# YiZhiXiaoGuLI/xerus

Hardware: AMD Instinct MI355X
Metric: GFLOP/s on TT contraction + TT-round sweep time, order-10 rank-256 (higher is better)
Workload: dtype f64; 1 GPU; TT order-10 n=20 rank-256: <x,y> + x.round(256) per step; order=10, mode_size=20, rank=256, parallelism=replicas x1

## Files before the change

### include/xerus_amd.h

```cpp
#ifndef XERUS_AMD_H
#define XERUS_AMD_H

#include <stddef.h>
#include <stdint.h>

#ifdef __cplusplus
extern "C" {
#endif

typedef struct xrs_handle_s* xrs_handle_t;

#define XRS_OK 0
#define XRS_EINVAL (-1)
#define XRS_ENOMEM (-2)
#define XRS_EHIP (-3)
#define XRS_ENUMERIC 1

int xrs_create(xrs_handle_t* handle, int device);
int xrs_destroy(xrs_handle_t handle);
int xrs_set_stream(xrs_handle_t handle, void* hip_stream);
void* xrs_get_stream(xrs_handle_t handle);
int xrs_synchronize(xrs_handle_t handle);
const char* xrs_last_error(void);
const char* xrs_version(void);

int xrs_malloc(xrs_handle_t handle, void** ptr, size_t bytes);
int xrs_free(xrs_handle_t handle, void* ptr);
size_t xrs_pool_bytes(xrs_handle_t handle);
int xrs_upload(xrs_handle_t handle, double* dst_dev, const double* src_host, size_t n);
int xrs_download(xrs_handle_t handle, double* dst_host, const double* src_dev, size_t n);
int xrs_memset_zero(xrs_handle_t handle, double* dst_dev, size_t n);
int xrs_copy(xrs_handle_t handle, double* dst_dev, const double* src_dev, size_t n);

int xrs_nrm2(xrs_handle_t handle, double* result, const double* x, size_t n);
int xrs_dot(xrs_handle_t handle, double* result, const double* x, const double* y, size_t n);
int xrs_asum(xrs_handle_t handle, double* result, const double* x, size_t n);
int xrs_scal(xrs_handle_t handle, double* x, double alpha, size_t n);
int xrs_axpy(xrs_handle_t handle, double* y, double alpha, const double* x, size_t n);
int xrs_scale_rows(xrs_handle_t handle, double* X, const double* s, size_t m, size_t n);

int xrs_gemm(xrs_handle_t handle, double* C, size_t M, size_t N, double alpha,
             const double* A, size_t lda, int transA, size_t K,
             const double* B, size_t ldb, int transB);

int xrs_gemm_batched(xrs_handle_t handle, size_t count, double* const* C, size_t M, size_t N, double alpha,
                     const double* const* A, size_t lda, int transA, size_t K,
                     const double* const* B, size_t ldb, int transB);

int xrs_gemm_sym(xrs_handle_t handle, double* C, size_t N, double alpha,
                 const double* A, size_t lda, int transA, size_t K,
                 const double* B, size_t ldb, int transB);

int xrs_gemm_forms(xrs_handle_t handle, size_t count, double* const* C, size_t M, size_t N, double alpha,
                   const double* const* A, size_t lda, int transA, size_t K,
                   const double* const* B, size_t ldb, int transB, int sym, int tri);

int xrs_gemm_f32(xrs_handle_t handle, float* C, size_t M, size_t N, float alpha,
                 const float* A, size_t lda, int transA, size_t K,
                 const float* B, size_t ldb, int transB);

int xrs_permute(xrs_handle_t handle, double* out, const double* in, size_t ndim,
                const size_t* dims, const size_t* shuffle);

int xrs_qc(xrs_handle_t handle, double* Q, double* C, size_t* rank, const double* A, size_t m, size_t n);
int xrs_cq(xrs_handle_t handle, double* C, double* Q, size_t* rank, const double* A, size_t m, size_t n);
int xrs_qr(xrs_handle_t handle, double* Q, double* R, const double* A, size_t m, size_t n);
int xrs_rq(xrs_handle_t handle, double* R, double* Q, const double* A, size_t m, size_t n);
int xrs_svd(xrs_handle_t handle, double* U, double* S, double* Vt, const double* A, size_t m, size_t n);
int xrs_svd_batched(xrs_handle_t handle, double* U, double* S, double* Vt, int* status,
                    const double* A, size_t batch, size_t m, size_t n);
int xrs_svd_batched_fits(size_t m, size_t n);
int xrs_solve(xrs_handle_t handle, double* X, const double* A, size_t m, size_t n, const double* B, size_t p);
int xrs_solve_least_squares(xrs_handle_t handle, double* X, const double* A, size_t m, size_t n, const double* B, size_t p);
int xrs_svd_rows_vt(xrs_handle_t handle, double* S, double* Vt, int* sweeps, const double* A, size_t p, size_t q, int kernel);
int xrs_sym_tridiag(xrs_handle_t handle, double* d, double* e, const double* A, size_t n);
int xrs_sym_eig_top(xrs_handle_t handle, double* lam, double* Ut, int* status, const double* A, size_t n, size_t kk);


int xrs_tt_move_core(xrs_handle_t handle, size_t d, const size_t* n, size_t* r, double** cores,
                     int canonicalized, size_t core_position, size_t position, int keep_rank);
int xrs_tt_round(xrs_handle_t handle, size_t d, const size_t* n, size_t* r, double** cores,
                 int canonicalized, size_t core_position, const size_t* max_ranks, double eps);
int xrs_tt_soft_threshold(xrs_handle_t handle, size_t d, const size_t* n, size_t* r, double** cores,
                          int canonicalized, size_t core_position, const double* taus);
int xrs_tt_entrywise_product(xrs_handle_t handle, size_t d, const size_t* ext, const size_t* ra, const double* const* A,
                             const size_t* rb, const double* const* B, double alpha, double** out);
int xrs_tt_entrywise_square(xrs_handle_t handle, size_t d, const size_t* ext, const size_t* r, const double* const* A,
                            double alpha, double** out, size_t* r_out);
int xrs_tt_rank_one_argmax(xrs_handle_t handle, size_t d, const size_t* ext, const double* const* cores, size_t* pos);
int xrs_tt_operator_apply(xrs_handle_t handle, size_t d, const size_t* n, const size_t* m, const size_t* p, const size_t* ra,
                          const double* const* A, const size_t* rb, const double* const* B, int transpose_a, double** out);
#define XRS_ROUND_CHAIN 1
#define XRS_ROUND_TRUNCATE 2
#define XRS_ROUND_REFERENCE 3
#define XRS_ROUND_GENERAL 4
int xrs_tt_last_round_path(xrs_handle_t handle);
int xrs_tt_dot(xrs_handle_t handle, double* result, size_t d, const size_t* n,
               const size_t* rx, const double* const* xcores,
               const size_t* ry, const double* const* ycores);

int xrs_tt_dot_async(xrs_handle_t handle, size_t d, const size_t* n,
                     const size_t* rx, const double* const* xcores,
                     const size_t* ry, const double* const* ycores);
int xrs_tt_dot_wait(xrs_handle_t handle, double* result);
int xrs_tt_dot_f32(xrs_handle_t handle, double* result, size_t d, const size_t* n,
                   const size_t* rx, const double* const* xcores,
                   const size_t* ry, const double* const* ycores);

int xrs_tt_tangent_project(xrs_handle_t handle, size_t d, const size_t* n, const size_t* ru, const double* const* U,
                           const size_t* rz, const double* const* Z, double** V, double** UU, size_t* fallback_edges);
int xrs_tt_tangent_to_tt(xrs_handle_t handle, size_t d, const size_t* n, const size_t* r, const double* const* U,
                         const double* const* V, int add_base, double** out);
int xrs_tt_tangent_dot(xrs_handle_t handle, double* result, size_t d, const size_t* n, const size_t* r,
                       const double* const* UU, const double* const* A, const double* const* B);

typedef int (*xrs_allreduce_fn)(void* ctx, double* buf, size_t count);
typedef int (*xrs_allgather_fn)(void* ctx, const double* send, double* recv, size_t count);

typedef struct xrs_comm_s* xrs_comm_t;
int xrs_comm_unique_id(void* id128_out);
int xrs_comm_create(xrs_handle_t handle, int nranks, int rank, const void* id128, xrs_comm_t* comm_out);
int xrs_comm_destroy(xrs_comm_t comm);
size_t xrs_comm_calls(xrs_comm_t comm);
int xrs_comm_allreduce(void* comm, double* buf, size_t count);
int xrs_comm_emulate(xrs_handle_t handle, int nranks, xrs_comm_t* comm_out);
int xrs_comm_allgather(void* comm, const double* send, double* recv, size_t count);

int xrs_tt_gather_sharded(xrs_handle_t handle, size_t d, const size_t* n_global, int world, int rank, const size_t* r,
                          const double* const* local_cores, double** full_cores_out, xrs_allgather_fn allgather, void* ctx);
int xrs_tt_shard(xrs_handle_t handle, size_t d, const size_t* n_global, int world, int rank, const size_t* r,
                 const double* const* full_cores, double** local_out);

int xrs_tt_round_sharded(xrs_handle_t handle, size_t d, const size_t* n_local, size_t* r, double** cores,
                         const size_t* max_ranks, double eps, xrs_allreduce_fn allreduce, void* ctx, int* certified);

int xrs_tt_round_sharded_ex(xrs_handle_t handle, size_t d, const size_t* n_local, size_t* r, double** cores,
                            const size_t* max_ranks, double eps, int world, int rank, xrs_allreduce_fn allreduce,
                            void* ctx, int* path);

int xrs_tt_dot_sharded(xrs_handle_t handle, double* result, size_t d, const size_t* n_local, const size_t* rx,
                       const double* const* X, const size_t* ry, const double* const* Y, xrs_allreduce_fn allreduce,
                       void* ctx);

int xrs_uq_basis(xrs_handle_t handle, double* P, const double* xi, size_t N, size_t n);
int xrs_uq_stack_congruence(xrs_handle_t handle, double* Lout, const double* Lprev, const double* X, const double* P,
                            size_t N, size_t a, size_t n, size_t b);
int xrs_uq_quadform(xrs_handle_t handle, double* result, const double* L, const double* V, size_t N, size_t a);


int xrs_philox_words(xrs_handle_t handle, uint32_t* out, size_t s, size_t q, uint64_t seed, uint32_t stream);
int xrs_gaussian_matrix(xrs_handle_t handle, double* G, size_t s, size_t m, uint64_t seed, uint32_t stream);
#define XRS_SKETCH_FUSED 1
#define XRS_SKETCH_MATERIALISED 2
int xrs_sketch_gaussian(xrs_handle_t handle, double* Y, size_t s, const double* A, size_t m, size_t n, uint64_t seed,
                        uint32_t stream, int route);
int xrs_sketch_last_route(xrs_handle_t handle);


int xrs_als_local_apply(xrs_handle_t handle, double* y, const double* x, size_t rl, size_t n, size_t rr, size_t pl,
                        size_t pr, const double* L, const double* A, const double* R, int normal);
#define XRS_CG_CONVERGED 0
#define XRS_CG_MAX_ITER 1
#define XRS_CG_BREAKDOWN 2
int xrs_als_local_cg(xrs_handle_t handle, double* x, const double* b, size_t rl, size_t n, size_t rr, size_t pl,
                     size_t pr, const double* L, const double* A, const double* R, int normal, double tol,
                     size_t max_iter, size_t check_every, size_t* iters, double* relres, int* status);

#define XRS_EIG_CONVERGED 0
#define XRS_EIG_MAX_ITER 1
#define XRS_EIG_BREAKDOWN 2
int xrs_als_local_eig(xrs_handle_t handle, double* x, size_t rl, size_t n, size_t rr, size_t pl, size_t pr,
                      const double* L, const double* A, const double* R, double tol, size_t max_iter, size_t check_every,
                      double* theta, size_t* iters, double* relres, int* status);
int xrs_geneig_lowest(int k, const double* G, const double* H, double* theta, double* c);

#define XRS_KFAM_GEMM 1u
#define XRS_KFAM_PERMUTE 2u
#define XRS_KFAM_QR 4u
#define XRS_KFAM_SVD 8u
#define XRS_KFAM_ELEMWISE 16u
#define XRS_KFAM_SPLITK 32u
int xrs_prof_begin(xrs_handle_t handle, uint32_t family_mask);
int xrs_prof_end(xrs_handle_t handle, size_t* launches, double* total_ms, double* flops, double* bytes);

#ifdef __cplusplus
}
#endif
#endif
```

### xerus_amd/capi.py

```python
from __future__ import annotations

import ctypes as C
import os
from typing import Sequence

import numpy as np

_HERE = os.path.dirname(os.path.abspath(__file__))
LIB_PATH = os.environ.get("XRS_LIB_PATH") or os.path.join(_HERE, "libxerus_amd.so")

_SZ = C.c_size_t
_DP = C.c_void_p

SIGNATURES = {
    "xrs_create": (C.c_int, [C.POINTER(_DP), C.c_int]),
    "xrs_destroy": (C.c_int, [_DP]),
    "xrs_set_stream": (C.c_int, [_DP, _DP]),
    "xrs_get_stream": (_DP, [_DP]),
    "xrs_synchronize": (C.c_int, [_DP]),
    "xrs_last_error": (C.c_char_p, []),
    "xrs_version": (C.c_char_p, []),
    "xrs_malloc": (C.c_int, [_DP, C.POINTER(_DP), _SZ]),
    "xrs_free": (C.c_int, [_DP, _DP]),
    "xrs_pool_bytes": (_SZ, [_DP]),
    "xrs_upload": (C.c_int, [_DP, _DP, _DP, _SZ]),
    "xrs_download": (C.c_int, [_DP, _DP, _DP, _SZ]),
    "xrs_memset_zero": (C.c_int, [_DP, _DP, _SZ]),
    "xrs_copy": (C.c_int, [_DP, _DP, _DP, _SZ]),
    "xrs_nrm2": (C.c_int, [_DP, C.POINTER(C.c_double), _DP, _SZ]),
    "xrs_dot": (C.c_int, [_DP, C.POINTER(C.c_double), _DP, _DP, _SZ]),
    "xrs_asum": (C.c_int, [_DP, C.POINTER(C.c_double), _DP, _SZ]),
    "xrs_scal": (C.c_int, [_DP, _DP, C.c_double, _SZ]),
    "xrs_axpy": (C.c_int, [_DP, _DP, C.c_double, _DP, _SZ]),
    "xrs_scale_rows": (C.c_int, [_DP, _DP, _DP, _SZ, _SZ]),
    "xrs_gemm": (C.c_int, [_DP, _DP, _SZ, _SZ, C.c_double, _DP, _SZ, C.c_int, _SZ, _DP, _SZ, C.c_int]),
    "xrs_gemm_f32": (C.c_int, [_DP, _DP, _SZ, _SZ, C.c_float, _DP, _SZ, C.c_int, _SZ, _DP, _SZ, C.c_int]),
    "xrs_gemm_sym": (C.c_int,[_DP, _DP, _SZ, C.c_double, _DP, _SZ, C.c_int, _SZ, _DP, _SZ, C.c_int]),
    "xrs_gemm_batched": (C.c_int, [_DP, _SZ, C.POINTER(_DP), _SZ, _SZ, C.c_double, C.POINTER(_DP), _SZ, C.c_int, _SZ,
                                   C.POINTER(_DP), _SZ, C.c_int]),
    "xrs_gemm_forms": (C.c_int, [_DP, _SZ, C.POINTER(_DP), _SZ, _SZ, C.c_double, C.POINTER(_DP), _SZ, C.c_int, _SZ,
                                 C.POINTER(_DP), _SZ, C.c_int, C.c_int, C.c_int]),
    "xrs_permute": (C.c_int, [_DP, _DP, _DP, _SZ, C.POINTER(_SZ), C.POINTER(_SZ)]),
    "xrs_qc": (C.c_int, [_DP, _DP, _DP, C.POINTER(_SZ), _DP, _SZ, _SZ]),
    "xrs_cq": (C.c_int, [_DP, _DP, _DP, C.POINTER(_SZ), _DP, _SZ, _SZ]),
    "xrs_qr": (C.c_int, [_DP, _DP, _DP, _DP, _SZ, _SZ]),
    "xrs_rq": (C.c_int, [_DP, _DP, _DP, _DP, _SZ, _SZ]),
    "xrs_svd": (C.c_int, [_DP, _DP, _DP, _DP, _DP, _SZ, _SZ]),
    "xrs_svd_batched": (C.c_int, [_DP, _DP, _DP, _DP, C.POINTER(C.c_int), _DP, _SZ, _SZ, _SZ]),
    "xrs_svd_batched_fits": (C.c_int, [_SZ, _SZ]),
    "xrs_solve": (C.c_int, [_DP, _DP, _DP, _SZ, _SZ, _DP, _SZ]),
    "xrs_solve_least_squares": (C.c_int, [_DP, _DP, _DP, _SZ, _SZ, _DP, _SZ]),
    "xrs_svd_rows_vt": (C.c_int, [_DP, _DP, _DP, C.POINTER(C.c_int), _DP, _SZ, _SZ, C.c_int]),
    "xrs_sym_eig_top": (C.c_int, [_DP, _DP, _DP, C.POINTER(C.c_int), _DP, _SZ, _SZ]),
    "xrs_sym_tridiag": (C.c_int, [_DP, _DP, _DP, _DP, _SZ]),
    "xrs_tt_entrywise_product": (C.c_int, [_DP, _SZ, C.POINTER(_SZ), C.POINTER(_SZ), C.POINTER(_DP), C.POINTER(_SZ), C.POINTER(_DP),
                                           C.c_double, C.POINTER(_DP)]),
    "xrs_tt_entrywise_square": (C.c_int, [_DP, _SZ, C.POINTER(_SZ), C.POINTER(_SZ), C.POINTER(_DP), C.c_double, C.POINTER(_DP),
                                          C.POINTER(_SZ)]),
    "xrs_tt_rank_one_argmax": (C.c_int, [_DP, _SZ, C.POINTER(_SZ), C.POINTER(_DP), C.POINTER(_SZ)]),
    "xrs_tt_operator_apply": (C.c_int, [_DP, _SZ, C.POINTER(_SZ), C.POINTER(_SZ), C.POINTER(_SZ), C.POINTER(_SZ), C.POINTER(_DP),
                                        C.POINTER(_SZ), C.POINTER(_DP), C.c_int, C.POINTER(_DP)]),
    "xrs_tt_move_core": (C.c_int, [_DP, _SZ, C.POINTER(_SZ), C.POINTER(_SZ), C.POINTER(_DP), C.c_int, _SZ, _SZ, C.c_int]),
    "xrs_tt_round": (C.c_int, [_DP, _SZ, C.POINTER(_SZ), C.POINTER(_SZ), C.POINTER(_DP), C.c_int, _SZ,
                               C.POINTER(_SZ), C.c_double]),
    "xrs_tt_dot": (C.c_int, [_DP, C.POINTER(C.c_double), _SZ, C.POINTER(_SZ), C.POINTER(_SZ), C.POINTER(_DP),
                             C.POINTER(_SZ), C.POINTER(_DP)]),
    "xrs_tt_dot_async": (C.c_int, [_DP, _SZ, C.POINTER(_SZ), C.POINTER(_SZ), C.POINTER(_DP), C.POINTER(_SZ),
                                   C.POINTER(_DP)]),
    "xrs_tt_dot_wait": (C.c_int, [_DP, C.POINTER(C.c_double)]),
    "xrs_tt_dot_f32": (C.c_int, [_DP, C.POINTER(C.c_double), _SZ, C.POINTER(_SZ), C.POINTER(_SZ), C.POINTER(_DP),
                                 C.POINTER(_SZ), C.POINTER(_DP)]),
    "xrs_tt_round_sharded": (C.c_int, [_DP, _SZ, C.POINTER(_SZ), C.POINTER(_SZ), C.POINTER(_DP), C.POINTER(_SZ),
                                       C.c_double, _DP, _DP, C.POINTER(C.c_int)]),
    "xrs_tt_round_sharded_ex": (C.c_int, [_DP, _SZ, C.POINTER(_SZ), C.POINTER(_SZ), C.POINTER(_DP), C.POINTER(_SZ),
                                          C.c_double, C.c_int, C.c_int, _DP, _DP, C.POINTER(C.c_int)]),
    "xrs_tt_dot_sharded": (C.c_int, [_DP, C.POINTER(C.c_double), _SZ, C.POINTER(_SZ), C.POINTER(_SZ), C.POINTER(_DP),
                                     C.POINTER(_SZ), C.POINTER(_DP), _DP, _DP]),
    "xrs_tt_tangent_project": (C.c_int, [_DP, _SZ, C.POINTER(_SZ), C.POINTER(_SZ), C.POINTER(_DP), C.POINTER(_SZ),
                                         C.POINTER(_DP), C.POINTER(_DP), C.POINTER(_DP), C.POINTER(_SZ)]),
    "xrs_tt_tangent_to_tt": (C.c_int, [_DP, _SZ, C.POINTER(_SZ), C.POINTER(_SZ), C.POINTER(_DP), C.POINTER(_DP), C.c_int,
                                       C.POINTER(_DP)]),
    "xrs_tt_tangent_dot": (C.c_int, [_DP, C.POINTER(C.c_double), _SZ, C.POINTER(_SZ), C.POINTER(_SZ), C.POINTER(_DP),
                                     C.POINTER(_DP), C.POINTER(_DP)]),
    "xrs_tt_last_round_path": (C.c_int, [_DP]),
    "xrs_tt_soft_threshold": (C.c_int, [_DP, _SZ, C.POINTER(_SZ), C.POINTER(_SZ), C.POINTER(_DP), C.c_int, _SZ,
                                        C.POINTER(C.c_double)]),
    "xrs_comm_unique_id": (C.c_int, [_DP]),
    "xrs_comm_create": (C.c_int, [_DP, C.c_int, C.c_int, _DP, C.POINTER(_DP)]),
    "xrs_comm_emulate": (C.c_int, [_DP, C.c_int, C.POINTER(_DP)]),
    "xrs_comm_destroy": (C.c_int, [_DP]),
    "xrs_comm_calls": (_SZ, [_DP]),
    "xrs_comm_allreduce": (C.c_int, [_DP, _DP, _SZ]),
    "xrs_comm_allgather": (C.c_int, [_DP, _DP, _DP, _SZ]),
    "xrs_tt_gather_sharded": (C.c_int, [_DP, _SZ, C.POINTER(_SZ), C.c_int, C.c_int, C.POINTER(_SZ), C.POINTER(_DP),
                                        C.POINTER(_DP), _DP, _DP]),
    "xrs_tt_shard": (C.c_int, [_DP, _SZ, C.POINTER(_SZ), C.c_int, C.c_int, C.POINTER(_SZ), C.POINTER(_DP), C.POINTER(_DP)]),
    "xrs_uq_basis": (C.c_int, [_DP, _DP, _DP, _SZ, _SZ]),
    "xrs_uq_stack_congruence": (C.c_int, [_DP, _DP, _DP, _DP, _DP, _SZ, _SZ, _SZ, _SZ]),
    "xrs_uq_quadform": (C.c_int, [_DP, C.POINTER(C.c_double), _DP, _DP, _SZ, _SZ]),
    "xrs_philox_words": (C.c_int, [_DP, _DP, _SZ, _SZ, C.c_uint64, C.c_uint32]),
    "xrs_gaussian_matrix": (C.c_int, [_DP, _DP, _SZ, _SZ, C.c_uint64, C.c_uint32]),
    "xrs_sketch_gaussian": (C.c_int, [_DP, _DP, _SZ, _DP, _SZ, _SZ, C.c_uint64, C.c_uint32, C.c_int]),
    "xrs_sketch_last_route": (C.c_int, [_DP]),
    "xrs_als_local_apply": (C.c_int, [_DP, _DP, _DP, _SZ, _SZ, _SZ, _SZ, _SZ, _DP, _DP, _DP, C.c_int]),
    "xrs_als_local_cg": (C.c_int, [_DP, _DP, _DP, _SZ, _SZ, _SZ, _SZ, _SZ, _DP, _DP, _DP, C.c_int, C.c_double, _SZ, _SZ,
                                   C.POINTER(_SZ), C.POINTER(C.c_double), C.POINTER(C.c_int)]),
    "xrs_als_local_eig": (C.c_int, [_DP, _DP, _SZ, _SZ, _SZ, _SZ, _SZ, _DP, _DP, _DP, C.c_double, _SZ, _SZ,
                                    C.POINTER(C.c_double), C.POINTER(_SZ), C.POINTER(C.c_double), C.POINTER(C.c_int)]),
    "xrs_geneig_lowest": (C.c_int, [C.c_int, C.POINTER(C.c_double), C.POINTER(C.c_double), C.POINTER(C.c_double),
                                    C.POINTER(C.c_double)]),
    "xrs_prof_begin": (C.c_int, [_DP, C.c_uint32]),
    "xrs_prof_end": (C.c_int, [_DP, C.POINTER(_SZ), C.POINTER(C.c_double), C.POINTER(C.c_double),
                               C.POINTER(C.c_double)]),
}

KFAM_GEMM, KFAM_PERMUTE, KFAM_QR, KFAM_SVD, KFAM_ELEMWISE, KFAM_SPLITK = 1, 2, 4, 8, 16, 32
ROUND_PATHS = {0: None, 1: "chain", 2: "truncate", 3: "reference", 4: "general"}
SKETCH_AUTO, SKETCH_FUSED, SKETCH_MATERIALISED = 0, 1, 2
SKETCH_ROUTES = {0: None, 1: "fused", 2: "materialised"}

_lib = None


class XrsError(RuntimeError):

    def __init__(self, fn: str, code: int, msg: str):
        super().__init__(f"{fn} failed with status {code}: {msg}")
        self.code = code


def load(path: str | None = None) -> C.CDLL:
    global _lib
    if _lib is not None and path is None:
        return _lib
    p = path or LIB_PATH
    if not os.path.exists(p):
        raise ImportError(f"{p} is missing: build it with `python -c 'import __graft_entry__ as g; g.build()'`")
    lib = C.CDLL(p)
    for name, (res, args) in SIGNATURES.items():
        f = getattr(lib, name)
        f.restype = res
        f.argtypes = args
    if path is None:
        _lib = lib
    return lib


def _check(fn: str, status: int):
    if status != 0:
        raise XrsError(fn, status, load().xrs_last_error().decode())


def svd_batched_fits(m: int, n: int) -> bool:
    return bool(load().xrs_svd_batched_fits(int(m), int(n)))


def geneig_lowest(k: int, G: Sequence[float], H: Sequence[float]):
    m = k * (k + 1) // 2
    if k not in (2, 3) or len(G) != m or len(H) != m:
        raise XrsError("xrs_geneig_lowest", -1, f"k = {k} needs {m} entries of each upper triangle")
    g, h = (C.c_double * m)(*[float(v) for v in G]), (C.c_double * m)(*[float(v) for v in H])
    theta, c = C.c_double(), (C.c_double * 3)()
    used = load().xrs_geneig_lowest(k, g, h, C.byref(theta), c)
    return used, theta.value, np.array(c[:k])


def _arr(vals: Sequence[int]):
    return (_SZ * len(vals))(*[int(v) for v in vals])


class Handle:

    def __init__(self, device: int = 0):
        self.lib = load()
        self.h = _DP()
        _check("xrs_create", self.lib.xrs_create(C.byref(self.h), device))

    def close(self):
        if self.h:
            _check("xrs_destroy", self.lib.xrs_destroy(self.h))
            self.h = _DP()

    def __del__(self):
        try:
            self.close()
        except Exception:
            pass

    def malloc(self, nbytes: int) -> int:
        p = _DP()
        _check("xrs_malloc", self.lib.xrs_malloc(self.h, C.byref(p), nbytes))
        return p.value or 0

    def free(self, ptr: int):
        _check("xrs_free", self.lib.xrs_free(self.h, _DP(ptr)))

    def pool_bytes(self) -> int:
        return int(self.lib.xrs_pool_bytes(self.h))

    def synchronize(self):
        _check("xrs_synchronize", self.lib.xrs_synchronize(self.h))

    def set_stream(self, stream_ptr: int | None):
        _check("xrs_set_stream", self.lib.xrs_set_stream(self.h, _DP(stream_ptr or 0)))

    def stream(self) -> int:
        return self.lib.xrs_get_stream(self.h) or 0

    def array(self, a: np.ndarray) -> "DeviceArray":
        return DeviceArray.from_host(self, a)

    def empty(self, shape) -> "DeviceArray":
        return DeviceArray(self, tuple(int(s) for s in shape))

    def zeros(self, shape) -> "DeviceArray":
        d = DeviceArray(self, tuple(int(s) for s in shape))
        _check("xrs_memset_zero", self.lib.xrs_memset_zero(self.h, _DP(d.ptr), d.size))
        return d

    def gemm(self, C_: "DeviceArray", M, N, alpha, A: "DeviceArray", lda, transA, K, B: "DeviceArray", ldb, transB):
        _check("xrs_gemm", self.lib.xrs_gemm(self.h, _DP(C_.ptr), M, N, alpha, _DP(A.ptr), lda, int(transA), K,
                                            _DP(B.ptr), ldb, int(transB)))

    def gemm_f32(self, C_: "Float32Array", M, N, alpha, A: "Float32Array", lda, transA, K, B: "Float32Array", ldb, transB):
        _check("xrs_gemm_f32", self.lib.xrs_gemm_f32(self.h, _DP(C_.ptr), M, N, float(alpha), _DP(A.ptr), lda, int(transA),
                                                    K, _DP(B.ptr), ldb, int(transB)))

    def array_f32(self, a: np.ndarray) -> "Float32Array":
        return Float32Array.from_host(self, a)

    def gemm_sym(self, C_: "DeviceArray", N, alpha, A: "DeviceArray", lda, transA, K, B: "DeviceArray", ldb, transB):
        _check("xrs_gemm_sym", self.lib.xrs_gemm_sym(self.h, _DP(C_.ptr), N, alpha, _DP(A.ptr), lda, int(transA), K,
                                                    _DP(B.ptr), ldb, int(transB)))

    def gemm_batched(self, Cs, M, N, alpha, As, lda, transA, K, Bs, ldb, transB):
        cnt = len(Cs)
        tab = lambda xs: (_DP * max(1, cnt))(*[_DP(x.ptr) for x in xs])
        _check("xrs_gemm_batched", self.lib.xrs_gemm_batched(self.h, cnt, tab(Cs), M, N, alpha, tab(As), lda, int(transA),
                                                            K, tab(Bs), ldb, int(transB)))

    def gemm_forms(self, Cs, M, N, alpha, As, lda, transA, K, Bs, ldb, transB, sym: bool = False, tri: int = 0):
        cnt = len(Cs)
        tab = lambda xs: (_DP * max(1, cnt))(*[_DP(x.ptr) for x in xs])
        _check("xrs_gemm_forms", self.lib.xrs_gemm_forms(self.h, cnt, tab(Cs), M, N, alpha, tab(As), lda, int(transA), K,
                                                        tab(Bs), ldb, int(transB), int(sym), int(tri)))

    def tangent_to_tt(self, n, r, Us, Vs, add_base: bool):
        d = len(n)
        tab = lambda xs: (_DP * d)(*[_DP(x.ptr) for x in xs])
        out = (_DP * d)()
        _check("xrs_tt_tangent_to_tt", self.lib.xrs_tt_tangent_to_tt(self.h, d, _arr(n), _arr(r), tab(Us), tab(Vs),
                                                                    int(add_base), out))
        cores = []
        for k in range(d):
            shape = (2 * r[k] if k else 1, n[k], 2 * r[k + 1] if k + 1 < d else 1)
            c = DeviceArray(self, shape, ptr=out[k])
            c.owned = True
            cores.append(c)
        return cores

    def matmul(self, A: "DeviceArray", transA: bool, B: "DeviceArray", transB: bool, alpha: float = 1.0):
        am, ak = (A.shape[1], A.shape[0]) if transA else (A.shape[0], A.shape[1])
        bk, bn = (B.shape[1], B.shape[0]) if transB else (B.shape[0], B.shape[1])
        assert ak == bk, (A.shape, B.shape)
        out = self.empty((am, bn))
        self.gemm(out, am, bn, alpha, A, A.shape[1], transA, ak, B, B.shape[1], transB)
        return out

    def permute(self, out: "DeviceArray", inp: "DeviceArray", dims, shuffle):
        _check("xrs_permute", self.lib.xrs_permute(self.h, _DP(out.ptr), _DP(inp.ptr), len(dims), _arr(dims),
                                                  _arr(shuffle)))

    def reshuffle(self, inp: "DeviceArray", shuffle):
        dims = inp.shape
        out_dims = [0] * len(dims)
        for i, s in enumerate(shuffle):
            out_dims[s] = dims[i]
        out = self.empty(tuple(out_dims))
        self.permute(out, inp, dims, shuffle)
        return out

    def nrm2(self, x: "DeviceArray") -> float:
        r = C.c_double()
        _check("xrs_nrm2", self.lib.xrs_nrm2(self.h, C.byref(r), _DP(x.ptr), x.size))
        return r.value

    def dot(self, x: "DeviceArray", y: "DeviceArray") -> float:
        r = C.c_double()
        _check("xrs_dot", self.lib.xrs_dot(self.h, C.byref(r), _DP(x.ptr), _DP(y.ptr), x.size))
        return r.value

    def asum(self, x: "DeviceArray") -> float:
        r = C.c_double()
        _check("xrs_asum", self.lib.xrs_asum(self.h, C.byref(r), _DP(x.ptr), x.size))
        return r.value

    def scal(self, x: "DeviceArray", alpha: float):
        _check("xrs_scal", self.lib.xrs_scal(self.h, _DP(x.ptr), alpha, x.size))

    def axpy(self, y: "DeviceArray", alpha: float, x: "DeviceArray"):
        _check("xrs_axpy", self.lib.xrs_axpy(self.h, _DP(y.ptr), alpha, _DP(x.ptr), x.size))

    def scale_rows(self, X: "DeviceArray", s: "DeviceArray"):
        _check("xrs_scale_rows", self.lib.xrs_scale_rows(self.h, _DP(X.ptr), _DP(s.ptr), X.shape[0], X.size // max(1, X.shape[0])))

    def qc(self, A: "DeviceArray"):
        m, n = A.shape
        k = min(m, n)
        Q, Cm = self.empty((m, k)), self.empty((k, n))
        r = _SZ()
        _check("xrs_qc", self.lib.xrs_qc(self.h, _DP(Q.ptr), _DP(Cm.ptr), C.byref(r), _DP(A.ptr), m, n))
        rank = r.value
        Q.shape, Cm.shape = (m, rank), (rank, n)
        return Q, Cm, rank

    def cq(self, A: "DeviceArray"):
        m, n = A.shape
        k = min(m, n)
        Cm, Q = self.empty((m, k)), self.empty((k, n))
        r = _SZ()
        _check("xrs_cq", self.lib.xrs_cq(self.h, _DP(Cm.ptr), _DP(Q.ptr), C.byref(r), _DP(A.ptr), m, n))
        rank = r.value
        Cm.shape, Q.shape = (m, rank), (rank, n)
        return Cm, Q, rank

    def qr(self, A: "DeviceArray"):
        m, n = A.shape
        k = min(m, n)
        Q, R = self.empty((m, k)), self.empty((k, n))
        _check("xrs_qr", self.lib.xrs_qr(self.h, _DP(Q.ptr), _DP(R.ptr), _DP(A.ptr), m, n))
        return Q, R

    def rq(self, A: "DeviceArray"):
        m, n = A.shape
        k = min(m, n)
        R, Q = self.empty((m, k)), self.empty((k, n))
        _check("xrs_rq", self.lib.xrs_rq(self.h, _DP(R.ptr), _DP(Q.ptr), _DP(A.ptr), m, n))
        return R, Q

    def svd(self, A: "DeviceArray"):
        m, n = A.shape
        k = min(m, n)
        U, S, Vt = self.empty((m, k)), self.empty((k,)), self.empty((k, n))
        _check("xrs_svd", self.lib.xrs_svd(self.h, _DP(U.ptr), _DP(S.ptr), _DP(Vt.ptr), _DP(A.ptr), m, n))
        return U, S, Vt

    def svd_batched(self, A: "DeviceArray", want_status: bool = True):
        batch, m, n = A.shape
        k = min(m, n)
        U, S, Vt = self.empty((batch, m, k)), self.empty((batch, k)), self.empty((batch, k, n))
        st = np.zeros(batch, dtype=np.intc) if want_status else None
        _check("xrs_svd_batched", self.lib.xrs_svd_batched(
            self.h, _DP(U.ptr), _DP(S.ptr), _DP(Vt.ptr), st.ctypes.data_as(C.POINTER(C.c_int)) if want_status else None,
            _DP(A.ptr), batch, m, n))
        return U, S, Vt, st

    def solve(self, A: "DeviceArray", B: "DeviceArray", least_squares: bool = False):
        m, n = A.shape
        p = B.shape[1] if len(B.shape) == 2 else 1
        X = self.empty((n, p) if len(B.shape) == 2 else (n,))
        fn = "xrs_solve_least_squares" if least_squares else "xrs_solve"
        _check(fn, getattr(self.lib, fn)(self.h, _DP(X.ptr), _DP(A.ptr), m, n, _DP(B.ptr), p))
        return X

    def sym_eig_top(self, A: "DeviceArray", kk: int):
        n = A.shape[0]
        lam, Ut, st = self.empty((kk,)), self.empty((kk, n)), C.c_int()
        _check("xrs_sym_eig_top", self.lib.xrs_sym_eig_top(self.h, _DP(lam.ptr), _DP(Ut.ptr), C.byref(st), _DP(A.ptr), n, kk))
        return lam, Ut, st.value

    def sym_tridiag(self, A: "DeviceArray"):
        n = A.shape[0]
        d, e = self.empty((n,)), self.empty((n,))
        _check("xrs_sym_tridiag", self.lib.xrs_sym_tridiag(self.h, _DP(d.ptr), _DP(e.ptr), _DP(A.ptr), n))
        return d.numpy(), e.numpy()[: n - 1]

    def svd_rows_vt(self, A: "DeviceArray", kernel: int = 0):
        p, q = A.shape
        S, Vt, sw = self.empty((p,)), self.empty((p, q)), C.c_int()
        _check("xrs_svd_rows_vt", self.lib.xrs_svd_rows_vt(self.h, _DP(S.ptr), _DP(Vt.ptr), C.byref(sw), _DP(A.ptr), p, q, kernel))
        return S, Vt, sw.value

    def tt_operator_apply(self, n, m, ra, A, rb, B, p=None, transpose=False):
        d = len(n)
        out = (_DP * d)()
        tab = lambda xs: (_DP * d)(*[_DP(x.ptr) for x in xs])
        _check("xrs_tt_operator_apply", self.lib.xrs_tt_operator_apply(
            self.h, d, _arr(n), _arr(m), _arr(p) if p is not None else None, _arr(ra), tab(A), _arr(rb), tab(B),
            int(transpose), out))
        res = []
        for k in range(d):
            nk = m[k] if transpose else n[k]
            shape = (ra[k] * rb[k], nk) + ((p[k],) if p is not None else ()) + (ra[k + 1] * rb[k + 1],)
            arr = DeviceArray(self, shape, ptr=out[k], owned=False)
            res.append(arr.numpy())
            self.free(out[k])
        return res

    def uq_basis(self, xi: "DeviceArray", n: int) -> "DeviceArray":
        N = xi.size
        P = self.empty((N, n))
        _check("xrs_uq_basis", self.lib.xrs_uq_basis(self.h, _DP(P.ptr), _DP(xi.ptr), N, n))
        return P

    def uq_stack_congruence(self, Lprev: "DeviceArray | None", X: "DeviceArray", P: "DeviceArray") -> "DeviceArray":
        a, n, b = X.shape
        N = P.shape[0]
        out = self.empty((N, b, b))
        _check("xrs_uq_stack_congruence", self.lib.xrs_uq_stack_congruence(
            self.h, _DP(out.ptr), _DP(Lprev.ptr) if Lprev is not None else None, _DP(X.ptr), _DP(P.ptr), N, a, n, b))
        return out

    def uq_quadform(self, L: "DeviceArray | None", V: "DeviceArray") -> float:
        N, a = V.shape
        r = C.c_double()
        _check("xrs_uq_quadform", self.lib.xrs_uq_quadform(self.h, C.byref(r), _DP(L.ptr) if L is not None else None,
                                                          _DP(V.ptr), N, a))
        return r.value

    @staticmethod
    def _seed_stream(fn: str, seed: int, stream: int):
        if not 0 <= int(seed) < 2 ** 64:
            raise XrsError(fn, -1, f"seed {seed} is not a 64-bit word")
        if not 0 <= int(stream) < 2 ** 32:
            raise XrsError(fn, -1, f"stream {stream} must be below 2^32")
        return int(seed), int(stream)

    def philox_words(self, s: int, q: int, seed: int, stream: int = 0) -> np.ndarray:
        seed, stream = self._seed_stream("xrs_philox_words", seed, stream)
        legal = 0 < s <= 2 ** 32 and q > 0
        buf = self.empty((2 * s * q,)) if legal else None
        _check("xrs_philox_words", self.lib.xrs_philox_words(self.h, _DP(buf.ptr) if legal else None, s, q, seed, stream))
        return buf.numpy().view(np.uint32).reshape(s, q, 4)

    def gaussian_matrix(self, s: int, m: int, seed: int, stream: int = 0) -> "DeviceArray":
        seed, stream = self._seed_stream("xrs_gaussian_matrix", seed, stream)
        legal = 0 < s <= 2 ** 32 and m > 0
        G = self.empty((s, m)) if legal else None
        _check("xrs_gaussian_matrix", self.lib.xrs_gaussian_matrix(self.h, _DP(G.ptr) if legal else None, s, m, seed, stream))
        return G

    def sketch_gaussian(self, s: int, A: "DeviceArray", seed: int, stream: int = 0, route: int = 0, m: int | None = None,
                        out: "DeviceArray | None" = None) -> "DeviceArray":
        seed, stream = self._seed_stream("xrs_sketch_gaussian", seed, stream)
        n = A.shape[1]
        m = A.shape[0] if m is None else int(m)
        legal = 0 < s <= 2 ** 32 and m > 0 and n > 0
        Y = out if out is not None else (self.empty((s, n)) if legal else None)
        _check("xrs_sketch_gaussian", self.lib.xrs_sketch_gaussian(self.h, _DP(Y.ptr) if Y is not None else None, s, _DP(A.ptr),
                                                                  m, n, seed, stream, int(route)))
        return Y

    def sketch_last_route(self) -> str | None:
        return SKETCH_ROUTES[self.lib.xrs_sketch_last_route(self.h)]

    @staticmethod
    def _local_extents(fn: str, dims, max_iter: int = 0, check_every: int = 1):
        for v in (*dims, max_iter, check_every):
            if not 0 <= int(v) < 2 ** 63:
                raise XrsError(fn, -1, f"extent or count {v} is not a size")
        return tuple(int(v) for v in dims)

    def als_local_apply(self, y: "DeviceArray | None", x: "DeviceArray | None", dims, L: "DeviceArray | None",
                        A: "DeviceArray | None", R: "DeviceArray | None", normal: bool):
        rl, n, rr, pl, pr = self._local_extents("xrs_als_local_apply", dims)
        ptr = lambda a: _DP(a.ptr) if a is not None else None
        _check("xrs_als_local_apply", self.lib.xrs_als_local_apply(self.h, ptr(y), ptr(x), rl, n, rr, pl, pr, ptr(L), ptr(A),
                                                                  ptr(R), int(bool(normal))))

    def als_local_cg(self, x: "DeviceArray | None", b: "DeviceArray | None", dims, L: "DeviceArray | None",
                     A: "DeviceArray | None", R: "DeviceArray | None", normal: bool, tol: float, max_iter: int = 0,
                     check_every: int = 1):
        rl, n, rr, pl, pr = self._local_extents("xrs_als_local_cg", dims, max_iter, check_every)
        ptr = lambda a: _DP(a.ptr) if a is not None else None
        iters, relres, status = _SZ(), C.c_double(), C.c_int()
        _check("xrs_als_local_cg", self.lib.xrs_als_local_cg(self.h, ptr(x), ptr(b), rl, n, rr, pl, pr, ptr(L), ptr(A), ptr(R),
                                                            int(bool(normal)), float(tol), int(max_iter), int(check_every),
                                                            C.byref(iters), C.byref(relres), C.byref(status)))
        return iters.value, relres.value, status.value

    def als_local_eig(self, x: "DeviceArray | None", dims, L: "DeviceArray | None", A: "DeviceArray | None",
                      R: "DeviceArray | None", tol: float, max_iter: int = 0, check_every: int = 1):
        rl, n, rr, pl, pr = self._local_extents("xrs_als_local_eig", dims, max_iter, check_every)
        ptr = lambda a: _DP(a.ptr) if a is not None else None
        theta, iters, relres, status = C.c_double(), _SZ(), C.c_double(), C.c_int()
        _check("xrs_als_local_eig", self.lib.xrs_als_local_eig(self.h, ptr(x), rl, n, rr, pl, pr, ptr(L), ptr(A), ptr(R),
                                                              float(tol), int(max_iter), int(check_every), C.byref(theta),
                                                              C.byref(iters), C.byref(relres), C.byref(status)))
        return theta.value, iters.value, relres.value, status.value

    def last_round_path(self) -> str | None:
        return ROUND_PATHS[self.lib.xrs_tt_last_round_path(self.h)]

    def prof_begin(self, mask: int):
        _check("xrs_prof_begin", self.lib.xrs_prof_begin(self.h, mask))

    def prof_end(self):
        n, ms, fl, by = _SZ(), C.c_double(), C.c_double(), C.c_double()
        _check("xrs_prof_end", self.lib.xrs_prof_end(self.h, C.byref(n), C.byref(ms), C.byref(fl), C.byref(by)))
        return {"launches": n.value, "ms": ms.value, "flops": fl.value, "bytes": by.value}


class DeviceArray:

    def __init__(self, handle: Handle, shape: tuple, ptr: int | None = None, owned: bool = True):
        self.handle = handle
        self.shape = tuple(shape)
        self.capacity = self.size
        self.owned = owned and ptr is None
        self.ptr = ptr if ptr is not None else (handle.malloc(max(8, self.capacity * 8)))

    @property
    def size(self) -> int:
        return int(np.prod(self.shape)) if self.shape else 1

    @classmethod
    def from_host(cls, handle: Handle, a: np.ndarray) -> "DeviceArray":
        a = np.ascontiguousarray(a, dtype=np.float64)
        d = cls(handle, a.shape)
        if a.size:
            _check("xrs_upload", handle.lib.xrs_upload(handle.h, _DP(d.ptr), a.ctypes.data_as(_DP), a.size))
        return d

    def numpy(self) -> np.ndarray:
        out = np.empty(self.shape, dtype=np.float64)
        assert self.size <= self.capacity, "shape exceeds the allocation"
        if self.size:
            _check("xrs_download", self.handle.lib.xrs_download(self.handle.h, out.ctypes.data_as(_DP), _DP(self.ptr),
                                                               self.size))
        return out

    def free(self):
        if self.owned and self.ptr:
            self.handle.free(self.ptr)
        self.ptr = 0

    def __del__(self):
        try:
            self.free()
        except Exception:
            pass


class Float32Array:

    def __init__(self, handle: Handle, shape: tuple, offset: int = 0):
        self.handle = handle
        self.shape = tuple(int(s) for s in shape)
        self.offset = int(offset)
        self._words = max(1, (self.size + self.offset + 1) // 2)
        self.base = handle.malloc(8 * self._words)
        self.ptr = self.base + 4 * self.offset

    @property
    def size(self) -> int:
        return int(np.prod(self.shape)) if self.shape else 1

    @classmethod
    def from_host(cls, handle: Handle, a: np.ndarray, offset: int = 0) -> "Float32Array":
        a = np.ascontiguousarray(a, dtype=np.float32)
        d = cls(handle, a.shape, offset)
        buf = np.zeros(2 * d._words, dtype=np.float32)
        buf[d.offset:d.offset + a.size] = a.ravel()
        _check("xrs_upload", handle.lib.xrs_upload(handle.h, _DP(d.base), buf.view(np.float64).ctypes.data_as(_DP), d._words))
        return d

    def numpy(self) -> np.ndarray:
        buf = np.empty(self._words, dtype=np.float64)
        _check("xrs_download", self.handle.lib.xrs_download(self.handle.h, buf.ctypes.data_as(_DP), _DP(self.base), self._words))
        return buf.view(np.float32)[self.offset:self.offset + self.size].reshape(self.shape).copy()

    def free(self):
        if self.base:
            self.handle.free(self.base)
        self.base = self.ptr = 0

    def __del__(self):
        try:
            self.free()
        except Exception:
            pass


class DotFuture:

    def __init__(self, handle: Handle):
        self.handle = handle
        self._value = None

    def result(self) -> float:
        if self._value is None:
            out = C.c_double()
            _check("xrs_tt_dot_wait", self.handle.lib.xrs_tt_dot_wait(self.handle.h, C.byref(out)))
            self._value = out.value
        return self._value


class TTDevice:

    def __init__(self, handle: Handle, dims, ranks, ptrs, canonicalized=False, core_position=0):
        self.handle = handle
        self.dims = [int(x) for x in dims]
        self.r = [int(x) for x in ranks]
        self.ptrs = list(ptrs)
        self.canonicalized = canonicalized
        self.core_position = core_position

    @classmethod
    def from_cores(cls, handle: Handle, cores, canonicalized=False, core_position=0) -> "TTDevice":
        dims = [c.shape[1] for c in cores]
        ranks = [cores[0].shape[0]] + [c.shape[2] for c in cores]
        ptrs = []
        for c in cores:
            c = np.ascontiguousarray(c, dtype=np.float64)
            p = handle.malloc(max(8, c.size * 8))
            _check("xrs_upload", handle.lib.xrs_upload(handle.h, _DP(p), c.ctypes.data_as(_DP), c.size))
            ptrs.append(p)
        return cls(handle, dims, ranks, ptrs, canonicalized, core_position)

    def clone(self) -> "TTDevice":
        ptrs = []
        for k, p in enumerate(self.ptrs):
            size = self.r[k] * self.dims[k] * self.r[k + 1]
            q = self.handle.malloc(max(8, size * 8))
            _check("xrs_copy", self.handle.lib.xrs_copy(self.handle.h, _DP(q), _DP(p), size))
            ptrs.append(q)
        return TTDevice(self.handle, self.dims, self.r, ptrs, self.canonicalized, self.core_position)

    @property
    def order(self):
        return len(self.dims)

    @property
    def ranks(self):
        return self.r[1:-1]

    def cores(self):
        out = []
        for k, p in enumerate(self.ptrs):
            shp = (self.r[k], self.dims[k], self.r[k + 1])
            a = np.empty(shp)
            _check("xrs_download", self.handle.lib.xrs_download(self.handle.h, a.ctypes.data_as(_DP), _DP(p), a.size))
            out.append(a)
        return out

    def _arrays(self):
        c = getattr(self, "_cache", None)
        if c is not None and c[3] is self.r and c[4] is self.ptrs:
            return c[0], c[1], c[2]
        d = self.order
        n = _arr(self.dims)
        r = _arr(self.r)
        cores = (_DP * d)(*self.ptrs)
        self._cache = (n, r, cores, self.r, self.ptrs)
        return n, r, cores

    def _writeback(self, r, cores):
        self.r = r[:]
        self.ptrs = [p or 0 for p in cores[:]]
        c = getattr(self, "_cache", None)
        if c is not None and c[1] is r and c[2] is cores:
            self._cache = (c[0], r, cores, self.r, self.ptrs)

    def move_core(self, position: int, keep_rank: bool = False):
        n, r, cores = self._arrays()
        st = self.handle.lib.xrs_tt_move_core(self.handle.h, self.order, n, r, cores, int(self.canonicalized),
                                              self.core_position, position, int(keep_rank))
        self._writeback(r, cores)
        _check("xrs_tt_move_core", st)
        self.canonicalized, self.core_position = True, position

    def round(self, max_ranks, eps: float = 8 * np.finfo(float).eps):
        d = self.order
        if isinstance(max_ranks, (int, np.integer)):
            max_ranks = [int(max_ranks)] * (d - 1)
        n, r, cores = self._arrays()
        key = tuple(max_ranks)
        mc = getattr(self, "_mr_cache", None)
        if mc is None or mc[0] != key:
            mc = (key, _arr(list(max_ranks) + [1]))
            self._mr_cache = mc
        mr = mc[1]
        st = self.handle.lib.xrs_tt_round(self.handle.h, d, n, r, cores, int(self.canonicalized), self.core_position,
                                          mr, eps)
        self._writeback(r, cores)
        _check("xrs_tt_round", st)
        self.canonicalized, self.core_position = True, 0

    def soft_threshold(self, taus):
        d = self.order
        if isinstance(taus, (int, float)):
            taus = [float(taus)] * (d - 1)
        n, r, cores = self._arrays()
        t = (C.c_double * max(1, d - 1))(*taus)
        st = self.handle.lib.xrs_tt_soft_threshold(self.handle.h, d, n, r, cores, int(self.canonicalized),
                                                   self.core_position, t)
        self._writeback(r, cores)
        _check("xrs_tt_soft_threshold", st)
        self.canonicalized, self.core_position = True, 0

    def dot(self, other: "TTDevice") -> float:
        if self.dims != other.dims:
            raise ValueError(f"dot of TTs with different dimensions: {self.dims} vs {other.dims}")
        out = C.c_double()
        n, rx, xc = self._arrays()
        _, ry, yc = other._arrays()
        _check("xrs_tt_dot", self.handle.lib.xrs_tt_dot(self.handle.h, C.byref(out), self.order, n, rx, xc, ry, yc))
        return out.value

    def dot_f32(self, other: "TTDevice") -> float:
        if self.dims != other.dims:
            raise ValueError(f"dot of TTs with different dimensions: {self.dims} vs {other.dims}")
        out = C.c_double()
        n, rx, xc = self._arrays()
        _, ry, yc = other._arrays()
        _check("xrs_tt_dot_f32", self.handle.lib.xrs_tt_dot_f32(self.handle.h, C.byref(out), self.order, n, rx, xc, ry, yc))
        return out.value

    def dot_async(self, other: "TTDevice") -> "DotFuture":
        if self.dims != other.dims:
            raise ValueError(f"dot of TTs with different dimensions: {self.dims} vs {other.dims}")
        if other.handle is not self.handle:
            raise ValueError("dot_async: both TTs must live on the same handle")
        n, rx, xc = self._arrays()
        _, ry, yc = other._arrays()
        _check("xrs_tt_dot_async", self.handle.lib.xrs_tt_dot_async(self.handle.h, self.order, n, rx, xc, ry, yc))
        return DotFuture(self.handle)

    def entrywise_square(self, alpha: float = 1.0) -> "TTDevice":
        d = self.order
        n, r, cores = self._arrays()
        out, r_out = (_DP * d)(), (_SZ * (d + 1))()
        _check("xrs_tt_entrywise_square", self.handle.lib.xrs_tt_entrywise_square(self.handle.h, d, n, r, cores, float(alpha),
                                                                                  out, r_out))
        return TTDevice(self.handle, self.dims, list(r_out), [p or 0 for p in out])

    def rank_one_argmax(self) -> list:
        if any(x != 1 for x in self.r):
            raise ValueError(f"rank_one_argmax needs ranks 1, got {self.r}")
        d = self.order
        n, _, cores = self._arrays()
        pos = (_SZ * d)()
        _check("xrs_tt_rank_one_argmax", self.handle.lib.xrs_tt_rank_one_argmax(self.handle.h, d, n, cores, pos))
        return [int(p) for p in pos]

    def frob_norm(self) -> float:
        if self.canonicalized:
            k = self.core_position
            size = self.r[k] * self.dims[k] * self.r[k + 1]
            return self.handle.nrm2(DeviceArray(self.handle, (size,), ptr=self.ptrs[k], owned=False))
        return float(np.sqrt(max(0.0, self.dot(self))))

    def free(self):
        for p in self.ptrs:
            if p:
                self.handle.free(p)
        self.ptrs = [0] * len(self.ptrs)

    def __del__(self):
        try:
            self.free()
        except Exception:
            pass
```

### xerus_amd/csrc/linalg.hip

```cpp
#include <cmath>
#include <cstdio>
#include <cstdlib>

#include "scratch_map.hpp"
#include "smallla.hpp"

namespace xrs {

constexpr double kU = 1.1102230246251565e-16;
constexpr double kDblEps = 2.220446049250313e-16;

void transpose(xrs_handle_t h, double* out, const double* in, size_t rows, size_t cols) {
    const size_t dims[2] = {rows, cols};
    const size_t shuf[2] = {1, 0};
    permute(h, out, in, 2, dims, shuf);
}

int read_status(xrs_handle_t h, const int* status_dev, int count, int* host_out) {
    int* hs = scratch::host<int>(h, scratch::kHostLocal, size_t(count));
    XRS_HIP(hipMemcpyAsync(hs, status_dev, size_t(count) * sizeof(int), hipMemcpyDeviceToHost, h->stream));
    XRS_HIP(hipStreamSynchronize(h->stream));
    int any = 0;
    for (int i = 0; i < count; ++i) {
        host_out[i] = hs[i];
        any |= hs[i];
    }
    return any;
}

__global__ void __launch_bounds__(256) k_dev_identity(const double* __restrict__ G, int n, double* __restrict__ out) {
    __shared__ double red[4];
    double mx = 0.0;
    for (int e = threadIdx.x; e < n * n; e += 256) {
        const double d = fabs(G[e] - ((e / n) == (e % n) ? 1.0 : 0.0));
        mx = (d > mx || d != d) ? d : mx;
    }
#pragma unroll
    for (int o = 32; o > 0; o >>= 1) {
        const double t = __shfl_xor(mx, o, 64);
        mx = (t > mx || t != t) ? t : mx;
    }
    if ((threadIdx.x & 63) == 0) red[threadIdx.x >> 6] = mx;
    __syncthreads();
    if (threadIdx.x == 0) {
        double m = red[0];
        for (int i = 1; i < 4; ++i) m = (red[i] > m || red[i] != red[i]) ? red[i] : m;
        out[0] = m;
    }
}

__global__ void __launch_bounds__(256) k_first_order(const double* __restrict__ G2, int n, double* __restrict__ L2,
                                                     double* __restrict__ Li2, double* __restrict__ emax) {
    __shared__ double red[4];
    double mx = 0.0;
    for (int e = threadIdx.x + blockIdx.x * 256; e < n * n; e += 256 * gridDim.x) {
        const int i = e / n, j = e % n;
        const double eij = G2[e] - (i == j ? 1.0 : 0.0);
        const double d = fabs(eij);
        mx = (d > mx || d != d) ? d : mx;
        const double el = (i > j) ? eij : ((i == j) ? 0.5 * eij : 0.0);
        L2[e] = (i == j ? 1.0 : 0.0) + el;
        Li2[e] = (i == j ? 1.0 : 0.0) - el;
    }
#pragma unroll
    for (int o = 32; o > 0; o >>= 1) {
        const double t = __shfl_xor(mx, o, 64);
        mx = (t > mx || t != t) ? t : mx;
    }
    if ((threadIdx.x & 63) == 0) red[threadIdx.x >> 6] = mx;
    __syncthreads();
    if (threadIdx.x == 0) {
        double m = red[0];
        for (int i = 1; i < 4; ++i) m = (red[i] > m || red[i] != red[i]) ? red[i] : m;
        emax[blockIdx.x] = m;
    }
}

static double max_abs_dev_identity(xrs_handle_t h, const double* G, size_t n) {
    double* out = scratch::dev<double>(h, scratch::kDevIdentityDev);
    hipLaunchKernelGGL(k_dev_identity, dim3(1), dim3(256), 0, h->stream, G, int(n), out);
    check_launch("k_dev_identity");
    double* hs = scratch::host<double>(h, scratch::kHostIdentityDev);
    XRS_HIP(hipMemcpyAsync(hs, out, 8, hipMemcpyDeviceToHost, h->stream));
    XRS_HIP(hipStreamSynchronize(h->stream));
    const double v = hs[0];
    return (v == v) ? v : 1e300;
}

static OrthResult orthogonalize_big(xrs_handle_t h, const double* A, size_t m, size_t n, bool wide, double* Q, double* RL) {
    const size_t N = wide ? m : n, M = wide ? n : m;
    OrthResult res{false, 0.0, false};
    const int nb = chol_full_blocks(N);
    DevBuf G(h, N * N * 8), L1(h, N * N * 8), Z1(h, N * N * 8), L2(h, N * N * 8), Z2(h, N * N * 8), L3(h, N * N * 8),
        Z3(h, N * N * 8), T(h, N * N * 8), Q1(h, m * n * 8), Q2(h, m * n * 8), st(h, size_t(3 * nb) * 4 + 64);
    auto gram = [&](double* out, const double* X) {
        if (wide) gemm_sym(h, out, N, 1.0, X, n, false, M, X, n, true);
        else gemm_sym(h, out, N, 1.0, X, n, true, M, X, n, false);
    };
    auto apply = [&](const double* Z, const double* X, double* out) {
        if (wide) gemm(h, out, N, n, 1.0, Z, N, false, N, X, n, false);
        else gemm(h, out, m, N, 1.0, X, n, false, N, Z, N, true);
    };
    auto all_zero = [&](int count) {
        std::vector<int> s(static_cast<size_t>(count));
        read_status(h, st.as<int>(), count, s.data());
        for (int v : s)
            if (v != 0) return false;
        return true;
    };
    const double tau_rel = 4.0 * double(M + 2 * N) * kU;
    gram(G.d(), A);
    chol_full(h, G.d(), N, -tau_rel, L1.d(), Z1.d(), st.as<int>());
    apply(Z1.d(), A, Q1.d());
    gram(G.d(), Q1.d());
    chol_full(h, G.d(), N, 0.0, L2.d(), Z2.d(), st.as<int>() + nb);
    apply(Z2.d(), Q1.d(), Q);
    if (wide) gemm(h, RL, N, N, 1.0, L1.d(), N, false, N, L2.d(), N, false);
    else gemm(h, RL, N, N, 1.0, L2.d(), N, true, N, L1.d(), N, true);
    if (all_zero(2 * nb)) {
        res.certified = true;
        res.cert_ratio = std::sqrt(0.5 * tau_rel);
        return res;
    }
    res.robust = true;
    const double s_rel = 11.0 * (double(M) * N + double(N) * (N + 1)) * kU;
    gram(G.d(), A);
    chol_full(h, G.d(), N, s_rel, L1.d(), Z1.d(), st.as<int>());
    apply(Z1.d(), A, Q1.d());
    gram(G.d(), Q1.d());
    chol_full(h, G.d(), N, 0.0, L2.d(), Z2.d(), st.as<int>() + nb);
    apply(Z2.d(), Q1.d(), Q2.d());
    gram(G.d(), Q2.d());
    chol_full(h, G.d(), N, 0.0, L3.d(), Z3.d(), st.as<int>() + 2 * nb);
    apply(Z3.d(), Q2.d(), Q);
    if (wide) {
        gemm(h, T.d(), N, N, 1.0, L1.d(), N, false, N, L2.d(), N, false);
        gemm(h, RL, N, N, 1.0, T.d(), N, false, N, L3.d(), N, false);
    } else {
        gemm(h, T.d(), N, N, 1.0, L3.d(), N, true, N, L2.d(), N, true);
        gemm(h, RL, N, N, 1.0, T.d(), N, false, N, L1.d(), N, true);
    }
    if (all_zero(3 * nb)) {
        gram(T.d(), Q);
        if (max_abs_dev_identity(h, T.d(), N) <= 64.0 * double(N) * kU) return res;
    }
    throw Error{XRS_ENUMERIC, "orthogonalize: a numerically rank-deficient matrix above 512 (shifted CholeskyQR3 failed)"};
}

OrthResult orthogonalize(xrs_handle_t h, const double* A, size_t m, size_t n, bool wide, double* Q, double* RL) {
    const size_t N = wide ? m : n;
    const size_t M = wide ? n : m;
    XRS_REQUIRE(N >= 1 && M >= N, "orthogonalize: need a tall (or, wide=true, a wide) matrix");
    OrthResult res{false, 0.0, false};
    if (N > size_t(kSmallMax)) return orthogonalize_big(h, A, m, n, wide, Q, RL);
    const int Ni = int(N), nvec = int(M);
    DevBuf G(h, N * N * 8), Dv(h, (N + 32) * 32 * 8), L1(h, N * N * 8), Q1(h, m * n * 8), st(h, 64);
    auto gram = [&](double* out, const double* X) {
        if (wide) gemm(h, out, N, N, 1.0, X, n, false, M, X, n, true);
        else gemm(h, out, N, N, 1.0, X, n, true, M, X, n, false);
    };
    auto solve = [&](const double* L, const double* Y, double* X) {
        trsm(h, wide, L, Dv.d(), Ni, Y, n, X, n, nvec);
    };
    const double tau_rel = 4.0 * double(M + 2 * N) * kU;
    int* stv = st.as<int>();
    gram(G.d(), A);
    potrf(h, G.d(), Ni, -tau_rel, Dv.d(), stv + 0);
    solve(G.d(), A, Q1.d());
    gram(L1.d(), Q1.d());
    {
        DevBuf L2(h, N * N * 8), Li2(h, N * N * 8);
        const unsigned nb = 8;
        double* emax_dev = scratch::dev<double>(h, scratch::kDevOrthEmax, nb);
        hipLaunchKernelGGL(k_first_order, dim3(nb), dim3(256), 0, h->stream, L1.d(), Ni, L2.d(), Li2.d(), emax_dev);
        check_launch("k_first_order");
        int* hs = scratch::host<int>(h, scratch::kHostResult, 2);
        double* hd = scratch::host<double>(h, scratch::kHostOrthEmax, nb);
        XRS_HIP(hipMemcpyAsync(hs, stv, 8, hipMemcpyDeviceToHost, h->stream));
        XRS_HIP(hipMemcpyAsync(hd, emax_dev, nb * 8, hipMemcpyDeviceToHost, h->stream));
        XRS_HIP(hipStreamSynchronize(h->stream));
        double em = 0.0;
        for (unsigned i = 0; i < nb; ++i) em = (hd[i] > em || hd[i] != hd[i]) ? hd[i] : em;
        if (hs[0] == 0 && em <= 1e-8) {
            if (wide) {
                gemm(h, Q, N, n, 1.0, Li2.d(), N, false, N, Q1.d(), n, false);
                gemm(h, RL, N, N, 1.0, G.d(), N, false, N, L2.d(), N, false);
            } else {
                gemm(h, Q, m, N, 1.0, Q1.d(), n, false, N, Li2.d(), N, true);
                gemm(h, RL, N, N, 1.0, L2.d(), N, true, N, G.d(), N, true);
            }
            res.certified = true;
            res.cert_ratio = std::sqrt(0.5 * tau_rel);
            return res;
        }
    }
    potrf(h, L1.d(), Ni, 0.0, Dv.d(), stv + 1);
    solve(L1.d(), Q1.d(), Q);
    if (wide) gemm(h, RL, N, N, 1.0, G.d(), N, false, N, L1.d(), N, false);
    else gemm(h, RL, N, N, 1.0, L1.d(), N, true, N, G.d(), N, true);
    int sts[3] = {0, 0, 0};
    if (read_status(h, stv, 2, sts) == 0) {
        res.certified = true;
        res.cert_ratio = std::sqrt(0.5 * tau_rel);
        return res;
    }
    res.robust = true;
    const double s_rel = 11.0 * (double(M) * N + double(N) * (N + 1)) * kU;
    DevBuf Q2(h, m * n * 8), L2(h, N * N * 8), T(h, N * N * 8);
    gram(G.d(), A);
    potrf(h, G.d(), Ni, s_rel, Dv.d(), stv + 0);
    solve(G.d(), A, Q1.d());
    gram(L1.d(), Q1.d());
    potrf(h, L1.d(), Ni, 0.0, Dv.d(), stv + 1);
    solve(L1.d(), Q1.d(), Q2.d());
    gram(L2.d(), Q2.d());
    potrf(h, L2.d(), Ni, 0.0, Dv.d(), stv + 2);
    solve(L2.d(), Q2.d(), Q);
    if (wide) {
        gemm(h, T.d(), N, N, 1.0, G.d(), N, false, N, L1.d(), N, false);
        gemm(h, RL, N, N, 1.0, T.d(), N, false, N, L2.d(), N, false);
    } else {
        gemm(h, T.d(), N, N, 1.0, L2.d(), N, true, N, L1.d(), N, true);
        gemm(h, RL, N, N, 1.0, T.d(), N, false, N, G.d(), N, true);
    }
    if (read_status(h, stv, 3, sts) == 0) {
        gram(T.d(), Q);
        if (max_abs_dev_identity(h, T.d(), N) <= 64.0 * double(N) * kU) return res;
    }
    if (!wide) {
        qrcp(h, A, m, n, Q, RL, false, false, false);
    } else {
        DevBuf At(h, m * n * 8), Qt(h, m * n * 8), Rt(h, m * m * 8);
        transpose(h, At.d(), A, m, n);
        qrcp(h, At.d(), n, m, Qt.d(), Rt.d(), false, false, false);
        transpose(h, Q, Qt.d(), n, m);
        transpose(h, RL, Rt.d(), m, m);
    }
    return res;
}

static bool small_problem(size_t m, size_t n) { return m * n <= 4096 || std::min(m, n) <= 8; }

static void compact_cols(xrs_handle_t h, double* dst, size_t ldd, const double* src, size_t lds, size_t rows, size_t cols) {
    if (ldd == lds && dst == src) return;
    XRS_HIP(hipMemcpy2DAsync(dst, ldd * 8, src, lds * 8, cols * 8, rows, hipMemcpyDeviceToDevice, h->stream));
}

static size_t qc_core(xrs_handle_t h, const double* A, size_t m, size_t n, double* Q, double* C) {
    const size_t k = std::min(m, n);
    auto exact = [&] {
        DevBuf Qf(h, m * k * 8);
        const size_t r = qrcp(h, A, m, n, Qf.d(), C, true, false, true);
        compact_cols(h, Q, r, Qf.d(), k, m, r);
        return r;
    };
    if (m < n || small_problem(m, n)) return exact();
    OrthResult o;
    try {
        o = orthogonalize(h, A, m, n, false, Q, C);
    } catch (const Error& e) {
        if (e.code != XRS_ENUMERIC) throw;
        return exact();
    }
    if (o.certified && o.cert_ratio > 64.0 * kDblEps) return n;
    return exact();
}

static size_t cq_core(xrs_handle_t h, const double* A, size_t m, size_t n, double* C, double* Q) {
    const size_t k = std::min(m, n);
    auto exact = [&] {
        DevBuf At(h, m * n * 8), Qt(h, n * k * 8), Ct(h, k * m * 8);
        transpose(h, At.d(), A, m, n);
        const size_t r = qrcp(h, At.d(), n, m, Qt.d(), Ct.d(), true, false, true);
        DevBuf Qc(h, n * r * 8 + 8);
        compact_cols(h, Qc.d(), r, Qt.d(), k, n, r);
        transpose(h, Q, Qc.d(), n, r);
        transpose(h, C, Ct.d(), r, m);
        return r;
    };
    if (n < m || small_problem(m, n)) return exact();
    OrthResult o;
    try {
        o = orthogonalize(h, A, m, n, true, Q, C);
    } catch (const Error& e) {
        if (e.code != XRS_ENUMERIC) throw;
        return exact();
    }
    if (o.certified && o.cert_ratio > 64.0 * kDblEps) return m;
    return exact();
}

static void qr_core(xrs_handle_t h, const double* A, size_t m, size_t n, double* Q, double* R) {
    if (m >= n && !small_problem(m, n)) {
        try {
            orthogonalize(h, A, m, n, false, Q, R);
            return;
        } catch (const Error& e) {
            if (e.code != XRS_ENUMERIC) throw;
        }
    }
    qrcp(h, A, m, n, Q, R, false, false, false);
}

static void rq_core(xrs_handle_t h, const double* A, size_t m, size_t n, double* R, double* Q) {
    if (m <= n && !small_problem(m, n)) {
        try {
            orthogonalize(h, A, m, n, true, Q, R);
            return;
        } catch (const Error& e) {
            if (e.code != XRS_ENUMERIC) throw;
        }
    }
    const size_t k = std::min(m, n);
    DevBuf At(h, m * n * 8), Qt(h, n * k * 8), Rt(h, k * m * 8);
    transpose(h, At.d(), A, m, n);
    qrcp(h, At.d(), n, m, Qt.d(), Rt.d(), false, false, false);
    transpose(h, Q, Qt.d(), n, k);
    transpose(h, R, Rt.d(), k, m);
}

template <class Run, class Back>
static auto range_controlled(xrs_handle_t h, const double* A, size_t count, Run run, Back scale_back) {
    double* am_dev = scratch::dev<double>(h, scratch::kDevRangeAmax);
    double* am_host = scratch::host<double>(h, scratch::kHostRangeAmax);
    amax_enqueue(h, &A, &count, 1, am_dev);
    XRS_HIP(hipMemcpyAsync(am_host, am_dev, 8, hipMemcpyDeviceToHost, h->stream));
    auto exponent = [&] { return range_exponent(am_host[0]); };
    decltype(run(A)) r{};
    try {
        r = run(A);
        if (exponent() == 0) return r;
    } catch (const Error&) {
        XRS_HIP(hipStreamSynchronize(h->stream));
        if (exponent() == 0) throw;
    }
    const int ex = exponent();
    DevBuf As(h, count * 8);
    ldexp_copy(h, As.d(), A, -ex, count);
    r = run(As.d());
    scale_back(r, ex);
    return r;
}

template <class Run>
static int range_scaled(xrs_handle_t h, const double* A, size_t count, Run run) {
    const int ex = range_exponent(h, A, count);
    DevBuf As(h, ex != 0 ? count * 8 : 0);
    if (ex != 0) ldexp_copy(h, As.d(), A, -ex, count);
    run(ex != 0 ? As.d() : A);
    return ex;
}

size_t qc(xrs_handle_t h, const double* A, size_t m, size_t n, double* Q, double* C) {
    XRS_REQUIRE(m > 0 && n > 0, "Dimension m and n must be larger than zero");
    return range_controlled(h, A, m * n, [&](const double* X) { return qc_core(h, X, m, n, Q, C); },
                            [&](size_t r, int ex) { ldexp_copy(h, C, C, ex, r * n); });
}

size_t cq(xrs_handle_t h, const double* A, size_t m, size_t n, double* C, double* Q) {
    XRS_REQUIRE(m > 0 && n > 0, "Dimension m and n must be larger than zero");
    return range_controlled(h, A, m * n, [&](const double* X) { return cq_core(h, X, m, n, C, Q); },
                            [&](size_t r, int ex) { ldexp_copy(h, C, C, ex, m * r); });
}

void qr(xrs_handle_t h, const double* A, size_t m, size_t n, double* Q, double* R) {
    XRS_REQUIRE(m > 0 && n > 0, "Dimension m and n must be larger than zero");
    range_controlled(h, A, m * n, [&](const double* X) { qr_core(h, X, m, n, Q, R); return 0; },
                     [&](int, int ex) { ldexp_copy(h, R, R, ex, std::min(m, n) * n); });
}

void rq(xrs_handle_t h, const double* A, size_t m, size_t n, double* R, double* Q) {
    XRS_REQUIRE(m > 0 && n > 0, "Dimension m and n must be larger than zero");
    range_controlled(h, A, m * n, [&](const double* X) { rq_core(h, X, m, n, R, Q); return 0; },
                     [&](int, int ex) { ldexp_copy(h, R, R, ex, m * std::min(m, n)); });
}

__global__ void k_div_cols(double* __restrict__ U, const double* __restrict__ S, size_t m, size_t k) {
    for (size_t e = size_t(blockIdx.x) * blockDim.x + threadIdx.x; e < m * k; e += size_t(gridDim.x) * blockDim.x) {
        const double s = S[e % k];
        U[e] = s > 0.0 ? U[e] / s : 0.0;
    }
}

static void svd_big(xrs_handle_t h, const double* A, size_t m, size_t n, double* U, double* S, double* Vt) {
    if (m < n) {
        DevBuf At(h, m * n * 8), U2(h, n * m * 8), V2(h, m * m * 8);
        transpose(h, At.d(), A, m, n);
        svd_big(h, At.d(), n, m, U2.d(), S, V2.d());
        transpose(h, U, V2.d(), m, m);
        transpose(h, Vt, U2.d(), n, m);
        return;
    }
    XRS_REQUIRE(n <= 1024, "svd: min(m, n) > 1024 not supported");
    DevBuf Q(h, m * n * 8), R(h, n * n * 8), Ur(h, n * n * 8), Uq(h, m * n * 8), Rn(h, n * n * 8), st(h, 64);
    orthogonalize(h, A, m, n, false, Q.d(), R.d());
    XRS_HIP(hipMemsetAsync(st.d(), 0, 64, h->stream));
    jacobi_vt(h, R.d(), int(n), false, int(n), int(n), S, Vt, int(n), st.as<int>(), 60);
    jacobi_settle(h, st.as<int>(), int(n), int(n), [&](int kernel) {
        jacobi_vt(h, R.d(), int(n), false, int(n), int(n), S, Vt, int(n), st.as<int>(), 60, kernel);
    });
    gemm(h, Ur.d(), n, n, 1.0, R.d(), n, false, n, Vt, n, true);
    hipLaunchKernelGGL(k_div_cols, dim3(unsigned(std::min<size_t>((n * n + 255) / 256, 4096))), dim3(256), 0, h->stream, Ur.d(), S, n, n);
    check_launch("k_div_cols");
    gemm(h, Uq.d(), m, n, 1.0, Q.d(), n, false, n, Ur.d(), n, false);
    orthogonalize(h, Uq.d(), m, n, false, U, Rn.d());
}

static void svd_core(xrs_handle_t h, const double* A, size_t m, size_t n, double* U, double* S, double* Vt);

static bool try_bidiag(xrs_handle_t h, const double* A, size_t n, double* U, double* S, double* Vt) {
    double diag[4];
    if (svd_bidiag(h, A, int(n), U, S, Vt, diag)) return true;
    if (svd_bidiag_mode() == 2) {
        char msg[200];
        std::snprintf(msg, sizeof msg, "svd_bidiag: check failed (residual %.3g, orthogonality %.3g / %.3g, status %d)", diag[0],
                      diag[1], diag[2], int(diag[3]));
        throw Error{XRS_ENUMERIC, msg};
    }
    return false;
}

void svd(xrs_handle_t h, const double* A, size_t m, size_t n, double* U, double* S, double* Vt) {
    XRS_REQUIRE(m > 0 && n > 0, "Dimension m and n must be larger than zero");
    if (m == n && n >= 16 && n <= 128 && svd_bidiag_mode() != 0 && try_bidiag(h, A, n, U, S, Vt)) return;
    const int ex = range_scaled(h, A, m * n, [&](const double* X) { svd_core(h, X, m, n, U, S, Vt); });
    ldexp_copy(h, S, S, ex, std::min(m, n));
}

static void svd_core(xrs_handle_t h, const double* A, size_t m, size_t n, double* U, double* S, double* Vt) {
    if (std::min(m, n) > size_t(kSmallMax)) {
        svd_big(h, A, m, n, U, S, Vt);
        return;
    }
    const size_t k = std::min(m, n);
    const bool bd = m != n && k >= 24 && k <= 128 && svd_bidiag_mode() != 0;
    if (!bd && m <= n && jacobi_usv_fits(int(m), int(n))) {
        jacobi_svd_rows(h, A, int(m), int(n), U, S, Vt);
        return;
    }
    DevBuf R(h, k * k * 8), Qf(h, m * n * 8), F(h, k * k * 8);
    if (m <= n) {
        rq_core(h, A, m, n, R.d(), Qf.d());
        if (!(bd && try_bidiag(h, R.d(), k, U, S, F.d()))) jacobi_svd_rows(h, R.d(), int(k), int(k), U, S, F.d());
        gemm(h, Vt, k, n, 1.0, F.d(), k, false, k, Qf.d(), n, false);
    } else {
        qr_core(h, A, m, n, Qf.d(), R.d());
        if (!(bd && try_bidiag(h, R.d(), k, F.d(), S, Vt))) jacobi_svd_rows(h, R.d(), int(k), int(k), F.d(), S, Vt);
        gemm(h, U, m, k, 1.0, Qf.d(), k, false, k, F.d(), k, false);
    }
}

}

using namespace xrs;

extern "C" {

int xrs_qc(xrs_handle_t h, double* Q, double* C, size_t* rank, const double* A, size_t m, size_t n) {
    return guarded([&] {
        XRS_REQUIRE(h && Q && C && rank && A, "null argument");
        fence_readers(h);
        *rank = qc(h, A, m, n, Q, C);
    });
}

int xrs_cq(xrs_handle_t h, double* C, double* Q, size_t* rank, const double* A, size_t m, size_t n) {
    return guarded([&] {
        XRS_REQUIRE(h && Q && C && rank && A, "null argument");
        fence_readers(h);
        *rank = cq(h, A, m, n, C, Q);
    });
}

int xrs_qr(xrs_handle_t h, double* Q, double* R, const double* A, size_t m, size_t n) {
    return guarded([&] {
        XRS_REQUIRE(h && Q && R && A, "null argument");
        fence_readers(h);
        qr(h, A, m, n, Q, R);
    });
}

int xrs_rq(xrs_handle_t h, double* R, double* Q, const double* A, size_t m, size_t n) {
    return guarded([&] {
        XRS_REQUIRE(h && Q && R && A, "null argument");
        fence_readers(h);
        rq(h, A, m, n, R, Q);
    });
}

int xrs_svd(xrs_handle_t h, double* U, double* S, double* Vt, const double* A, size_t m, size_t n) {
    return guarded([&] {
        XRS_REQUIRE(h && U && S && Vt && A, "null argument");
        fence_readers(h);
        svd(h, A, m, n, U, S, Vt);
    });
}

int xrs_sym_eig_top(xrs_handle_t h, double* lam, double* Ut, int* status, const double* A, size_t n, size_t kk) {
    return guarded([&] {
        XRS_REQUIRE(h && lam && Ut && status && A, "null argument");
        XRS_REQUIRE(n >= 2 && n <= 256 && kk >= 1 && kk <= n, "xrs_sym_eig_top: need 2 <= n <= 256 and 1 <= kk <= n");
        fence_readers(h);
        DevBuf st(h, 64);
        XRS_HIP(hipMemsetAsync(st.d(), 0, 64, h->stream));
        const int ex = range_scaled(h, A, n * n, [&](const double* X) {
            sym_eig_top(h, X, int(n), int(n), int(kk), lam, nullptr, Ut, int(n), st.as<int>());
        });
        ldexp_copy(h, lam, lam, ex, kk);
        read_status(h, st.as<int>(), 1, status);
    });
}

int xrs_sym_tridiag(xrs_handle_t h, double* d, double* e, const double* A, size_t n) {
    return guarded([&] {
        XRS_REQUIRE(h && d && e && A, "null argument");
        XRS_REQUIRE(n >= 2 && n <= 256, "xrs_sym_tridiag: need 2 <= n <= 256");
        fence_readers(h);
        sym_tridiag(h, A, int(n), int(n), d, e);
        XRS_HIP(hipStreamSynchronize(h->stream));
    });
}

int xrs_svd_rows_vt(xrs_handle_t h, double* S, double* Vt, int* sweeps, const double* A, size_t p, size_t q, int kernel) {
    return guarded([&] {
        XRS_REQUIRE(h && S && Vt && A && sweeps, "null argument");
        XRS_REQUIRE(p >= 1 && p <= q && q <= 1024 && (kernel != 1 || p <= 512),
                    "xrs_svd_rows_vt: need 1 <= p <= q <= 1024 (kernel 1: p <= 512)");
        DevBuf st(h, 64);
        XRS_HIP(hipMemsetAsync(st.d(), 0, 64, h->stream));
        const int ex = range_scaled(h, A, p * q, [&](const double* X) {
            jacobi_vt(h, X, int(q), false, int(p), int(q), S, Vt, int(q), st.as<int>(), 40, kernel, stamps_enabled("svd"));
        });
        ldexp_copy(h, S, S, ex, p);
        int sts[9];
        read_status(h, st.as<int>(), 9, sts);
        *sweeps = sts[0];
        if (stamps_enabled("svd"))
            std::fprintf(stderr, "jacobi_vt p=%zu q=%zu kernel=%d: sweeps %d, 100 MHz ticks: total %d, grid barriers %d, exchange %d; "
                         "thread-0 cross-round cycles: dot %d, rotation %d, update %d, barrier %d, rotations %d\n",
                         p, q, kernel, sts[0], sts[1], sts[2], sts[3], sts[4], sts[5], sts[6], sts[7], sts[8]);
    });
}

}
```

### xerus_amd/csrc/smallla.hip

```cpp
#include "smallla.hpp"

#include <cstdio>

namespace xrs {

constexpr int NB = 32;
typedef double d4 __attribute__((ext_vector_type(4)));
constexpr int PMAX = 512;
constexpr int POT_THREADS = 512;

__device__ __forceinline__ double readlane_d(double v, int l) {
    union { double d; int i[2]; } u;
    u.d = v;
    u.i[0] = __builtin_amdgcn_readlane(u.i[0], l);
    u.i[1] = __builtin_amdgcn_readlane(u.i[1], l);
    return u.d;
}

__device__ __forceinline__ void potrf32_body(double* __restrict__ G, int n, double shift_rel, double* __restrict__ Dinv,
                                             int* __restrict__ status, double* __restrict__ info,
                                             const double* src = nullptr) {
    __shared__ double P[PMAX * (NB + 1)];
    __shared__ double Ds[NB][NB + 1];
    __shared__ double red[16];
    __shared__ int fail;
    const int tid = threadIdx.x, lane = tid & 63, wave = tid >> 6;
    if (src != nullptr && src != G) {
        for (int e = tid; e < n * n; e += POT_THREADS) G[e] = src[e];
        __syncthreads();
    }
    double* dummy = Dinv + size_t(n + 31) * NB + (tid & 31);
    if (tid == 0) fail = 0;
    double tr = 0.0;
    for (int i = tid; i < n; i += POT_THREADS) tr += G[size_t(i) * n + i];
#pragma unroll
    for (int o = 32; o > 0; o >>= 1) tr += __shfl_xor(tr, o, 64);
    if (lane == 0) red[wave] = tr;
    __syncthreads();
    tr = 0.0;
    for (int w = 0; w < POT_THREADS / 64; ++w) tr += red[w];
    if (tid == 0 && info) info[0] = tr;
    const double shift = shift_rel * tr;
    if (shift != 0.0)
        for (int i = tid; i < n; i += POT_THREADS) G[size_t(i) * n + i] += shift;
    __syncthreads();
    for (int j0 = 0; j0 < n; j0 += NB) {
        const int jb = min(NB, n - j0);
        for (int e = tid; e < NB * NB; e += POT_THREADS) {
            const int r = e / NB, c = e % NB;
            double v = (r == c) ? 1.0 : 0.0;
            if (r < jb && c < jb && c <= r) v = G[size_t(j0 + r) * n + j0 + c];
            Ds[r][c] = v;
        }
        __syncthreads();
        if (wave == 0) {
            const int r = lane & 31;
            double row[NB];
#pragma unroll
            for (int c = 0; c < NB; ++c) row[c] = Ds[r][c];
            int bad = 0;
#pragma unroll
            for (int k = 0; k < NB; ++k) {
                double dkk = readlane_d(row[k], k);
                const bool okp = (dkk > 0.0) && (dkk < 1.0e300);
                if (!okp && bad == 0 && k < jb) bad = k + 1;
                if (!okp) dkk = 1.0;
                const double d = sqrt(dkk);
                const double inv = 1.0 / d;
                row[k] = (r == k) ? d : ((r > k) ? row[k] * inv : row[k]);
#pragma unroll
                for (int l = k + 1; l < NB; ++l) {
                    const double v = readlane_d(row[k], l);
                    if (r >= l) row[l] -= row[k] * v;
                }
            }
            if (lane < 32) {
#pragma unroll
                for (int c = 0; c < NB; ++c) Ds[r][c] = (c <= r) ? row[c] : 0.0;
            }
            if (lane == 0 && bad && fail == 0) fail = j0 + bad;
        }
        __syncthreads();
        const int t = n - j0 - jb;
        if (wave == 1) {
            const int c = lane & 31;
            double x[NB];
#pragma unroll
            for (int i = 0; i < NB; ++i) x[i] = (i == c) ? 1.0 : 0.0;
#pragma unroll
            for (int k = 0; k < NB; ++k) {
                x[k] = x[k] / Ds[k][k];
#pragma unroll
                for (int i = k + 1; i < NB; ++i) x[i] -= Ds[i][k] * x[k];
            }
            if (lane < 32) {
                double* out = Dinv + size_t(j0) * NB + c;
#pragma unroll
                for (int i = 0; i < NB; ++i) out[size_t(i) * NB] = x[i];
            }
        } else {
            const int wt = (tid >= 64) ? tid - 64 : tid;
            for (int e = wt; e < NB * NB; e += POT_THREADS - 64) {
                const int r = e / NB, c = e % NB;
                if (r < jb && c < jb && c <= r) G[size_t(j0 + r) * n + j0 + c] = Ds[r][c];
            }
            if (jb == NB) {
                for (int rr = wt; rr < t; rr += POT_THREADS - 64) {
                    double* grow = G + size_t(j0 + jb + rr) * n + j0;
                    int off = 0;
                    asm volatile("" : "+v"(off));
                    const double* D = &Ds[0][0] + off;
                    double x[NB];
#pragma unroll
                    for (int c = 0; c < NB; ++c) x[c] = grow[c];
#pragma unroll
                    for (int k = 0; k < NB; ++k) {
                        x[k] = x[k] / D[k * (NB + 1) + k];
#pragma unroll
                        for (int c = k + 1; c < NB; ++c) x[c] -= x[k] * D[c * (NB + 1) + k];
                    }
                    double* prow = P + rr * (NB + 1);
#pragma unroll
                    for (int c = 0; c < NB; ++c) {
                        prow[c] = x[c];
                        grow[c] = x[c];
                    }
                }
            } else {
                for (int rr = wt; rr < t; rr += POT_THREADS - 64) {
                    double* grow = G + size_t(j0 + jb + rr) * n + j0;
                    double* prow = P + rr * (NB + 1);
                    for (int c = 0; c < NB; ++c) prow[c] = (c < jb) ? grow[c] : 0.0;
                    for (int k = 0; k < jb; ++k) {
                        const double xk = prow[k] / Ds[k][k];
                        prow[k] = xk;
                        grow[k] = xk;
                        for (int c = k + 1; c < jb; ++c) prow[c] -= xk * Ds[c][k];
                    }
                }
            }
        }
        __syncthreads();
        if (t > 0) {
            const int T = (t + 15) / 16;
            const int ntiles = T * (T + 1) / 2;
            const int lr = lane & 15, lk = lane >> 4;
            for (int tile = wave; tile < ntiles; tile += POT_THREADS / 64) {
                int ti = int((sqrt(8.0 * tile + 1.0) - 1.0) * 0.5);
                while ((ti + 1) * (ti + 2) / 2 <= tile) ++ti;
                while (ti * (ti + 1) / 2 > tile) --ti;
                const int tk = tile - ti * (ti + 1) / 2;
                const int i0 = ti * 16, k0 = tk * 16;
                auto cptr = [&](int r) -> double* {
                    const int i = i0 + lk + 4 * r, k = k0 + lr;
                    const bool ok = (i < t) && (k < t);
                    return ok ? (G + size_t(j0 + jb + i) * n + j0 + jb + k) : dummy;
                };
                const double cv0 = *cptr(0), cv1 = *cptr(1), cv2 = *cptr(2), cv3 = *cptr(3);
                d4 acc = {0.0, 0.0, 0.0, 0.0};
                const int ra = min(i0 + lr, t - 1), rb = min(k0 + lr, t - 1);
#pragma unroll
                for (int c = 0; c < NB; c += 4) {
                    const double av = P[ra * (NB + 1) + c + lk];
                    const double bv = P[rb * (NB + 1) + c + lk];
                    acc = __builtin_amdgcn_mfma_f64_16x16x4f64(av, bv, acc, 0, 0, 0);
                }
                *cptr(0) = cv0 - acc[0];
                *cptr(1) = cv1 - acc[1];
                *cptr(2) = cv2 - acc[2];
                *cptr(3) = cv3 - acc[3];
            }
        }
        __syncthreads();
    }
    for (int e = tid; e < n * n; e += POT_THREADS) {
        const int r = e / n, c = e % n;
        if (c > r) G[size_t(r) * n + c] = 0.0;
    }
    if (tid == 0) status[0] = fail;
}

__global__ void __launch_bounds__(POT_THREADS) k_potrf(double* __restrict__ G, int n, double shift_rel, double* __restrict__ Dinv,
                                                 int* __restrict__ status, double* __restrict__ info) {
    potrf32_body(G, n, shift_rel, Dinv, status, info);
}

constexpr int PR_THREADS = 512;
constexpr int PR_WAVES = PR_THREADS / 64;
constexpr int PR_TMAX = 16;
constexpr int PR_SLOTS = (PR_TMAX * (PR_TMAX + 1) / 2 + PR_WAVES - 1) / PR_WAVES;
constexpr int PT = 17;
constexpr int PTILE = 16 * PT;

__device__ __forceinline__ double rsqrt_nr(double x) {
    double y = __builtin_amdgcn_rsq(x);
#pragma unroll
    for (int it = 0; it < 2; ++it) {
        const double e = fma(-x * y, y, 1.0);
        y = fma(0.5 * y, e, y);
    }
    return y;
}

__device__ __forceinline__ void wave_lds_sync() {
    __builtin_amdgcn_fence(__ATOMIC_RELEASE, "wavefront");
    __builtin_amdgcn_wave_barrier();
    __builtin_amdgcn_fence(__ATOMIC_ACQUIRE, "wavefront");
}

#ifdef XRS_POTRF_STAMPS
__device__ long long* g_potrf_stamps;
#define PSTAMP(i) do { if (threadIdx.x == 0) g_potrf_stamps[i] = __builtin_amdgcn_s_memtime(); } while (0)
#else
#define PSTAMP(i) do { } while (0)
#endif
template <int K>
__device__ __forceinline__ double row_bcast_d(double v) {
    union { double d; int i[2]; } u;
    u.d = v;
    u.i[0] = __builtin_amdgcn_mov_dpp(u.i[0], 0x150 + K, 0xF, 0xF, false);
    u.i[1] = __builtin_amdgcn_mov_dpp(u.i[1], 0x150 + K, 0xF, 0xF, false);
    return u.d;
}

template <int K>
__device__ __forceinline__ void factor_step(double (&a)[16], double (&w)[4], double* dsh, int lane, int valid, int& bad) {
    const double dkk = row_bcast_d<K>(a[K]);
    if (!((dkk > 0.0) && (dkk < 1.0e300)) && bad == 0 && K < valid) bad = K + 1;
    if (lane == 0) dsh[K] = dkk;
    double r = __builtin_amdgcn_rcp(dkk);
    r = fma(r, fma(-dkk, r, 1.0), r);
    r = fma(r, fma(-dkk, r, 1.0), r);
    const double m = a[K] * r;
#pragma unroll
    for (int l = K + 1; l < 16; ++l) a[l] = fma(-m, row_bcast_d<K>(a[l]), a[l]);
    const double mm = ((lane & 15) > K) ? m : 0.0;
#pragma unroll
    for (int t = 0; t < 4; ++t) w[t] = fma(-mm, row_bcast_d<K>(w[t]), w[t]);
}

template <int K>
__device__ __forceinline__ void factor_all(double (&a)[16], double (&w)[4], double* dsh, int lane, int valid, int& bad) {
    if constexpr (K < 16) {
        factor_step<K>(a, w, dsh, lane, valid, bad);
        factor_all<K + 1>(a, w, dsh, lane, valid, bad);
    }
}

__device__ __forceinline__ int diag_factor16(double* Dt, double* Di, double* dsh, double* __restrict__ dinv_out,
                                             int lane, int valid) {
    const int r = lane & 15, g = lane >> 4;
    double a[16], w[4];
#pragma unroll
    for (int c = 0; c < 16; ++c) a[c] = Dt[r * PT + c];
#pragma unroll
    for (int t = 0; t < 4; ++t) w[t] = (g + 4 * t == r) ? 1.0 : 0.0;
    int bad = 0;
    factor_all<0>(a, w, dsh, lane, valid, bad);
    wave_lds_sync();
#ifdef XRS_POTRF_STAMPS
    if (lane == 0) g_potrf_stamps[1000 + blockIdx.x] = __builtin_amdgcn_s_memtime();
#endif
    if (lane < 16) {
#pragma unroll
        for (int c = 0; c < 16; ++c) Dt[r * PT + c] = (c <= r) ? a[c] : 0.0;
    }
    const double rsr = rsqrt_nr(dsh[r]);
#pragma unroll
    for (int t = 0; t < 4; ++t) {
        const double v = w[t] * rsr;
        Di[r * PT + g + 4 * t] = v;
        dinv_out[r * 16 + g + 4 * t] = v;
    }
    wave_lds_sync();
#pragma unroll
    for (int e = 0; e < 4; ++e) {
        const int rr = lane >> 2, cc = 4 * (lane & 3) + e;
        if (cc <= rr) Dt[rr * PT + cc] *= rsqrt_nr(dsh[cc]);
    }
    wave_lds_sync();
    return bad;
}

template <int P>
__device__ __forceinline__ void trail_pair(d4 (&acc)[PR_SLOTS], const int (&ti)[PR_SLOTS], const int (&tk)[PR_SLOTS], int j,
                                           const double* Pbuf, int oa) {
    const bool hi = tk[P] > j;
    bool lo = false;
    if constexpr (P > 0) lo = tk[P - 1] > j;
    if (!hi && !lo) return;
    auto op = [&](int tile, int c) -> double {
        return *reinterpret_cast<const double*>(reinterpret_cast<const char*>(Pbuf + max(tile, 0) * PTILE) + oa + 32 * c);
    };
    double a1[4], b1[4];
#pragma unroll
    for (int c = 0; c < 4; ++c) {
        a1[c] = hi ? -op(ti[P], c) : 0.0;
        b1[c] = hi ? op(tk[P], c) : 0.0;
    }
    if constexpr (P > 0) {
        double a0[4], b0[4];
#pragma unroll
        for (int c = 0; c < 4; ++c) {
            a0[c] = lo ? -op(ti[P - 1], c) : 0.0;
            b0[c] = lo ? op(tk[P - 1], c) : 0.0;
        }
#pragma unroll
        for (int c = 0; c < 4; ++c) {
            acc[P] = __builtin_amdgcn_mfma_f64_16x16x4f64(a1[c], b1[c], acc[P], 0, 0, 0);
            acc[P - 1] = __builtin_amdgcn_mfma_f64_16x16x4f64(a0[c], b0[c], acc[P - 1], 0, 0, 0);
        }
    } else {
#pragma unroll
        for (int c = 0; c < 4; ++c) acc[P] = __builtin_amdgcn_mfma_f64_16x16x4f64(a1[c], b1[c], acc[P], 0, 0, 0);
    }
}

template <int P>
__device__ __forceinline__ void trail_all(d4 (&acc)[PR_SLOTS], const int (&ti)[PR_SLOTS], const int (&tk)[PR_SLOTS], int j,
                                          const double* Pbuf, int oa) {
    if constexpr (P >= 0) {
        trail_pair<P>(acc, ti, tk, j, Pbuf, oa);
        trail_all<P - 2>(acc, ti, tk, j, Pbuf, oa);
    }
}

__device__ __forceinline__ void potrf_rr_body(double* __restrict__ G, int n, double shift_rel, double* __restrict__ Dinv,
                                              int* __restrict__ status, double* __restrict__ info,
                                              const double* __restrict__ src = nullptr) {
    const double* __restrict__ S = src != nullptr ? src : G;
    __shared__ double Dt[PTILE];
    __shared__ double Di[PTILE];
    __shared__ double P[PR_TMAX * PTILE];
    __shared__ double ivs[16];
    __shared__ double red[PR_WAVES];
    __shared__ int fail;
    const int tid = threadIdx.x, lane = tid & 63;
    const int wave = __builtin_amdgcn_readfirstlane(tid >> 6);
    const int lr = lane & 15, lg = lane >> 4;
    const int T = (n + 15) >> 4;
    const int ntiles = T * (T + 1) / 2;
    if (tid == 0) fail = 0;
    PSTAMP(0);
    double tr = 0.0;
    for (int i = tid; i < n; i += PR_THREADS) tr += S[size_t(i) * n + i];
#pragma unroll
    for (int o = 32; o > 0; o >>= 1) tr += __shfl_xor(tr, o, 64);
    if (lane == 0) red[wave] = tr;
    __syncthreads();
    tr = 0.0;
#pragma unroll
    for (int w = 0; w < PR_WAVES; ++w) tr += red[w];
    if (tid == 0 && info) info[0] = tr;
    const double shift = shift_rel * tr;

    int ti[PR_SLOTS], tk[PR_SLOTS];
    d4 acc[PR_SLOTS];
#pragma unroll
    for (int s = 0; s < PR_SLOTS; ++s) {
        const int t = s * PR_WAVES + wave;
        int i = -1, k = -1;
        if (t < ntiles) {
            int start = 0;
            k = 0;
            while (t >= start + (T - k)) { start += T - k; ++k; }
            i = k + (t - start);
        }
        ti[s] = i;
        tk[s] = k;
#pragma unroll
        for (int q = 0; q < 4; ++q) {
            const int row = min(max(16 * i + lg + 4 * q, 0), n - 1), col = min(max(16 * k + lr, 0), n - 1);
            acc[s][q] = S[size_t(row) * n + col];
        }
    }
#pragma unroll
    for (int s = 0; s < PR_SLOTS; ++s)
#pragma unroll
        for (int q = 0; q < 4; ++q) {
            const int row = 16 * ti[s] + lg + 4 * q, col = 16 * tk[s] + lr;
            const bool inside = ti[s] >= 0 && row < n && col < n;
            const double pad = (row == col) ? 1.0 : 0.0;
            acc[s][q] = inside ? acc[s][q] + ((row == col) ? shift : 0.0) : pad;
        }

    for (int j = 0; j < T; ++j) {
        int oc = (lg * PT + lr) * 8, oa = (lr * PT + lg) * 8;
        asm volatile("" : "+v"(oc), "+v"(oa));
        auto cpos = [&](double* base, int q) -> double* {
            return reinterpret_cast<double*>(reinterpret_cast<char*>(base) + oc) + 4 * q * PT;
        };
        auto apos = [&](const double* base, int c) -> const double* {
            return reinterpret_cast<const double*>(reinterpret_cast<const char*>(base) + oa) + 4 * c;
        };
#pragma unroll
        for (int s = 0; s < PR_SLOTS; ++s)
            if (ti[s] == j && tk[s] == j) {
#pragma unroll
                for (int q = 0; q < 4; ++q) *cpos(Dt, q) = acc[s][q];
            }
        __syncthreads();
        PSTAMP(2 + 4 * j);
        if (wave == 0) {
            const int bad = diag_factor16(Dt, Di, ivs, Dinv + size_t(j) * 256, lane, n - 16 * j);
            if (lane == 0 && bad && fail == 0) fail = 16 * j + bad;
        }
        __syncthreads();
        PSTAMP(3 + 4 * j);
#pragma unroll
        for (int s = 0; s < PR_SLOTS; ++s) {
            if (tk[s] != j) continue;
            if (ti[s] == j) {
#pragma unroll
                for (int q = 0; q < 4; ++q) acc[s][q] = *cpos(Dt, q);
                continue;
            }
            double* Pi = P + ti[s] * PTILE;
#pragma unroll
            for (int q = 0; q < 4; ++q) *cpos(Pi, q) = acc[s][q];
            wave_lds_sync();
            d4 rr = {0.0, 0.0, 0.0, 0.0};
#pragma unroll
            for (int c = 0; c < 4; ++c) rr = __builtin_amdgcn_mfma_f64_16x16x4f64(*apos(Pi, c), *apos(Di, c), rr, 0, 0, 0);
            wave_lds_sync();
#pragma unroll
            for (int q = 0; q < 4; ++q) *cpos(Pi, q) = rr[q];
            acc[s] = rr;
        }
        __syncthreads();
        PSTAMP(4 + 4 * j);
        trail_all<PR_SLOTS - 1>(acc, ti, tk, j, P, oa);
    }
    __syncthreads();
    PSTAMP(1);
    int sg = lg, sr = lr;
    asm volatile("" : "+v"(sg), "+v"(sr));
#pragma unroll
    for (int s = 0; s < PR_SLOTS; ++s) {
        if (ti[s] < 0 || G == nullptr) continue;
#pragma unroll
        for (int q = 0; q < 4; ++q) {
            const int row = 16 * ti[s] + sg + 4 * q, col = 16 * tk[s] + sr;
            if (row < n && col < n) {
                G[size_t(row) * n + col] = (col <= row) ? acc[s][q] : 0.0;
                if (ti[s] != tk[s]) G[size_t(col) * n + row] = 0.0;
            }
        }
    }
    __syncthreads();
    if (tid == 0) status[0] = fail;
}

constexpr int LA_THREADS = PR_THREADS;
constexpr int LA_WAVES = LA_THREADS / 64;
constexpr int LA_SLOTS = PR_SLOTS;

template <int P>
__device__ __forceinline__ void la_trail_pair(d4 (&acc)[LA_SLOTS], const int (&ti)[LA_SLOTS], const int (&tk)[LA_SLOTS],
                                              int kmin, int kmax, const double* Pbuf, int oa) {
    const bool hi = tk[P] >= kmin && tk[P] <= kmax;
    bool lo = false;
    if constexpr (P > 0) lo = tk[P - 1] >= kmin && tk[P - 1] <= kmax;
    if (!hi && !lo) return;
    auto op = [&](int tile, int c) -> double {
        return *reinterpret_cast<const double*>(reinterpret_cast<const char*>(Pbuf + max(tile, 0) * PTILE) + oa + 32 * c);
    };
    double a1[4], b1[4];
#pragma unroll
    for (int c = 0; c < 4; ++c) {
        a1[c] = hi ? -op(ti[P], c) : 0.0;
        b1[c] = hi ? op(tk[P], c) : 0.0;
    }
    if constexpr (P > 0) {
        double a0[4], b0[4];
#pragma unroll
        for (int c = 0; c < 4; ++c) {
            a0[c] = lo ? -op(ti[P - 1], c) : 0.0;
            b0[c] = lo ? op(tk[P - 1], c) : 0.0;
        }
#pragma unroll
        for (int c = 0; c < 4; ++c) {
            acc[P] = __builtin_amdgcn_mfma_f64_16x16x4f64(a1[c], b1[c], acc[P], 0, 0, 0);
            acc[P - 1] = __builtin_amdgcn_mfma_f64_16x16x4f64(a0[c], b0[c], acc[P - 1], 0, 0, 0);
        }
    } else {
#pragma unroll
        for (int c = 0; c < 4; ++c) acc[P] = __builtin_amdgcn_mfma_f64_16x16x4f64(a1[c], b1[c], acc[P], 0, 0, 0);
    }
}

template <int P>
__device__ __forceinline__ void la_trail_all(d4 (&acc)[LA_SLOTS], const int (&ti)[LA_SLOTS], const int (&tk)[LA_SLOTS],
                                             int kmin, int kmax, const double* Pbuf, int oa) {
    if constexpr (P >= 0) {
        la_trail_pair<P>(acc, ti, tk, kmin, kmax, Pbuf, oa);
        la_trail_all<P - 2>(acc, ti, tk, kmin, kmax, Pbuf, oa);
    }
}

__device__ __forceinline__ void potrf_la_body(double* __restrict__ G, int n, double shift_rel, double* __restrict__ Dinv,
                                              int* __restrict__ status, double* __restrict__ info,
                                              const double* __restrict__ src = nullptr) {
    const double* __restrict__ S = src != nullptr ? src : G;
    __shared__ double Dt[PTILE];
    __shared__ double Di[PTILE];
    __shared__ double P[PR_TMAX * PTILE];
    __shared__ double ivs[16];
    __shared__ double red[LA_WAVES];
    __shared__ int fail;
    const int tid = threadIdx.x, lane = tid & 63;
    const int wave = __builtin_amdgcn_readfirstlane(tid >> 6);
    const int lr = lane & 15, lg = lane >> 4;
    const int T = (n + 15) >> 4;
    const int ntiles = T * (T + 1) / 2;
    if (tid == 0) fail = 0;
    PSTAMP(0);
    double tr = 0.0;
    for (int i = tid; i < n; i += LA_THREADS) tr += S[size_t(i) * n + i];
#pragma unroll
    for (int o = 32; o > 0; o >>= 1) tr += __shfl_xor(tr, o, 64);
    if (lane == 0) red[wave] = tr;
    __syncthreads();
    tr = 0.0;
#pragma unroll
    for (int w = 0; w < LA_WAVES; ++w) tr += red[w];
    if (tid == 0 && info) info[0] = tr;
    const double shift = shift_rel * tr;

    int ti[LA_SLOTS], tk[LA_SLOTS];
    d4 acc[LA_SLOTS];
#pragma unroll
    for (int s = 0; s < LA_SLOTS; ++s) {
        const int t = wave == 0 ? s : LA_SLOTS + s * (LA_WAVES - 1) + (wave - 1);
        int i = -1, k = -1;
        if (t < ntiles) {
            int start = 0;
            k = 0;
            while (t >= start + (T - k)) { start += T - k; ++k; }
            i = k + (t - start);
        }
        ti[s] = i;
        tk[s] = k;
#pragma unroll
        for (int q = 0; q < 4; ++q) {
            const int row = min(max(16 * i + lg + 4 * q, 0), n - 1), col = min(max(16 * k + lr, 0), n - 1);
            acc[s][q] = S[size_t(row) * n + col];
        }
    }
#pragma unroll
    for (int s = 0; s < LA_SLOTS; ++s)
#pragma unroll
        for (int q = 0; q < 4; ++q) {
            const int row = 16 * ti[s] + lg + 4 * q, col = 16 * tk[s] + lr;
            const bool inside = ti[s] >= 0 && row < n && col < n;
            const double pad = (row == col) ? 1.0 : 0.0;
            acc[s][q] = inside ? acc[s][q] + ((row == col) ? shift : 0.0) : pad;
        }

    int oc = (lg * PT + lr) * 8, oa = (lr * PT + lg) * 8;
    auto cpos = [&](double* base, int q) -> double* {
        return reinterpret_cast<double*>(reinterpret_cast<char*>(base) + oc) + 4 * q * PT;
    };
    auto apos = [&](const double* base, int c) -> const double* {
        return reinterpret_cast<const double*>(reinterpret_cast<const char*>(base) + oa) + 4 * c;
    };
    auto publish_diag = [&](int j) {
#pragma unroll
        for (int s = 0; s < LA_SLOTS; ++s)
            if (ti[s] == j && tk[s] == j) {
#pragma unroll
                for (int q = 0; q < 4; ++q) *cpos(Dt, q) = acc[s][q];
            }
    };
    auto factor_diag = [&](int j) {
        if (wave == 0) {
            const int bad = diag_factor16(Dt, Di, ivs, Dinv + size_t(j) * 256, lane, n - 16 * j);
            if (lane == 0 && bad && fail == 0) fail = 16 * j + bad;
        }
    };
    publish_diag(0);
    __syncthreads();
    factor_diag(0);
    __syncthreads();
    for (int j = 0; j < T; ++j) {
        asm volatile("" : "+v"(oc), "+v"(oa));
        PSTAMP(2 + 4 * j);
#pragma unroll
        for (int s = 0; s < LA_SLOTS; ++s) {
            if (tk[s] != j) continue;
            if (ti[s] == j) {
#pragma unroll
                for (int q = 0; q < 4; ++q) acc[s][q] = *cpos(Dt, q);
                continue;
            }
            double* Pi = P + ti[s] * PTILE;
#pragma unroll
            for (int q = 0; q < 4; ++q) *cpos(Pi, q) = acc[s][q];
            wave_lds_sync();
            d4 rr = {0.0, 0.0, 0.0, 0.0};
#pragma unroll
            for (int c = 0; c < 4; ++c) rr = __builtin_amdgcn_mfma_f64_16x16x4f64(*apos(Pi, c), *apos(Di, c), rr, 0, 0, 0);
            wave_lds_sync();
#pragma unroll
            for (int q = 0; q < 4; ++q) *cpos(Pi, q) = rr[q];
            acc[s] = rr;
        }
        __syncthreads();
        if (j + 1 >= T) break;
        PSTAMP(3 + 4 * j);
        la_trail_all<LA_SLOTS - 1>(acc, ti, tk, j + 1, j + 1, P, oa);
        publish_diag(j + 1);
        __syncthreads();
        PSTAMP(4 + 4 * j);
        if (wave == 0) factor_diag(j + 1);
        la_trail_all<LA_SLOTS - 1>(acc, ti, tk, j + 2, T - 1, P, oa);
        __syncthreads();
    }
    PSTAMP(1);
    int sg = lg, sr = lr;
    asm volatile("" : "+v"(sg), "+v"(sr));
#pragma unroll
    for (int s = 0; s < LA_SLOTS; ++s) {
        if (ti[s] < 0 || G == nullptr) continue;
#pragma unroll
        for (int q = 0; q < 4; ++q) {
            const int row = 16 * ti[s] + sg + 4 * q, col = 16 * tk[s] + sr;
            if (row < n && col < n) {
                G[size_t(row) * n + col] = (col <= row) ? acc[s][q] : 0.0;
                if (ti[s] != tk[s]) G[size_t(col) * n + row] = 0.0;
            }
        }
    }
    __syncthreads();
    if (tid == 0) status[0] = fail;
}

#ifdef XRS_POTRF_NO_LOOKAHEAD
#define XRS_POTRF_RR_BODY potrf_rr_body
#else
#define XRS_POTRF_RR_BODY potrf_la_body
#endif
#define XRS_POTRF_RR_THREADS PR_THREADS
__global__ void __launch_bounds__(XRS_POTRF_RR_THREADS) k_potrf_rr(double* __restrict__ G, int n, double shift_rel,
                                                         double* __restrict__ Dinv, int* __restrict__ status,
                                                         double* __restrict__ info) {
    XRS_POTRF_RR_BODY(G, n, shift_rel, Dinv, status, info);
}

__global__ void __launch_bounds__(POT_THREADS) k_potrf32_batched(PotrfBatch b) {
    const int i = blockIdx.x;
    potrf32_body(b.G[i], b.n[i], b.shift[i], b.Dinv[i], b.status + b.slot[i], nullptr, b.src[i]);
}

__global__ void __launch_bounds__(XRS_POTRF_RR_THREADS) k_potrf_rr_batched(PotrfBatch b) {
    const int i = blockIdx.x;
    XRS_POTRF_RR_BODY(b.G[i], b.n[i], b.shift[i], b.Dinv[i], b.status + b.slot[i], nullptr, b.src[i]);
}

template <bool COLS, int TMAX>
__device__ __forceinline__ void trsm16_body(const double* __restrict__ L, const double* __restrict__ Dinv, int dld,
                                            int n, const double* __restrict__ Y, size_t ldy, double* __restrict__ X,
                                            size_t ldx, int nvec, int v0, bool ident) {
    constexpr int JS = TMAX / 4;
    __shared__ double Xs[TMAX * 16 * PT];
    __shared__ double red[2][4][256];
    const int tid = threadIdx.x, lane = tid & 63;
    const int wave = __builtin_amdgcn_readfirstlane(tid >> 6);
    const int lr = lane & 15, lg = lane >> 4;
    const int T = (n + 15) >> 4;
    const int np = T * 16;
    for (int e = tid; e < np * 16; e += 256) {
        int i, v;
        if (COLS) { i = e >> 4; v = e & 15; } else { v = e / np; i = e - v * np; }
        double y = 0.0;
        if (i < n && v0 + v < nvec) {
            if (ident) y = (i == v0 + v) ? 1.0 : 0.0;
            else y = COLS ? Y[size_t(i) * ldy + v0 + v] : Y[size_t(v0 + v) * ldy + i];
        }
        Xs[i * PT + v] = y;
    }
    auto dinv_at = [&](int I, int c) -> double {
        const int off = (dld == 32) ? 16 * (I & 1) : 0;
        return Dinv[size_t(16 * I + lr) * dld + off + 4 * c + lg];
    };
    d4 xr[JS];
    double la[JS][4], lb[JS][4], da[4], db[4];
#pragma unroll
    for (int js = 0; js < JS; ++js) {
        xr[js] = d4{0.0, 0.0, 0.0, 0.0};
#pragma unroll
        for (int c = 0; c < 4; ++c) la[js][c] = 0.0;
    }
#pragma unroll
    for (int c = 0; c < 4; ++c) da[c] = dinv_at(0, c);
    __syncthreads();
    for (int I = 0; I < T; ++I) {
        if (I + 1 < T) {
            const int row = 16 * (I + 1) + lr;
#pragma unroll
            for (int js = 0; js < JS; ++js) {
                const int J = wave + 4 * js;
#pragma unroll
                for (int c = 0; c < 4; ++c)
                    lb[js][c] = (J <= I && row < n) ? L[size_t(row) * n + 16 * J + 4 * c + lg] : 0.0;
            }
#pragma unroll
            for (int c = 0; c < 4; ++c) db[c] = dinv_at(I + 1, c);
        }
        d4 y;
#pragma unroll
        for (int q = 0; q < 4; ++q) y[q] = Xs[(16 * I + lg + 4 * q) * PT + lr];
        d4 accj[JS];
#pragma unroll
        for (int js = 0; js < JS; ++js) {
            accj[js] = d4{0.0, 0.0, 0.0, 0.0};
            if (wave + 4 * js >= I) continue;
#pragma unroll
            for (int c = 0; c < 4; ++c) accj[js] = __builtin_amdgcn_mfma_f64_16x16x4f64(la[js][c], xr[js][c], accj[js], 0, 0, 0);
        }
        d4 acc = accj[0];
#pragma unroll
        for (int js = 1; js < JS; ++js) acc += accj[js];
        double* rb = red[I & 1][0];
#pragma unroll
        for (int q = 0; q < 4; ++q) rb[wave * 256 + q * 64 + lane] = acc[q];
        __syncthreads();
        d4 t;
#pragma unroll
        for (int q = 0; q < 4; ++q)
            t[q] = y[q] - ((rb[q * 64 + lane] + rb[256 + q * 64 + lane]) + (rb[512 + q * 64 + lane] + rb[768 + q * 64 + lane]));
        d4 x0 = {0.0, 0.0, 0.0, 0.0}, x1 = {0.0, 0.0, 0.0, 0.0};
        x0 = __builtin_amdgcn_mfma_f64_16x16x4f64(da[0], t[0], x0, 0, 0, 0);
        x1 = __builtin_amdgcn_mfma_f64_16x16x4f64(da[1], t[1], x1, 0, 0, 0);
        x0 = __builtin_amdgcn_mfma_f64_16x16x4f64(da[2], t[2], x0, 0, 0, 0);
        x1 = __builtin_amdgcn_mfma_f64_16x16x4f64(da[3], t[3], x1, 0, 0, 0);
        const d4 x = x0 + x1;
        if ((I & 3) == wave) {
#pragma unroll
            for (int js = 0; js < JS; ++js)
                if (js == (I >> 2)) xr[js] = x;
#pragma unroll
            for (int q = 0; q < 4; ++q) Xs[(16 * I + lg + 4 * q) * PT + lr] = x[q];
        }
#pragma unroll
        for (int js = 0; js < JS; ++js)
#pragma unroll
            for (int c = 0; c < 4; ++c) la[js][c] = lb[js][c];
#pragma unroll
        for (int c = 0; c < 4; ++c) da[c] = db[c];
    }
    __syncthreads();
    for (int e = tid; e < np * 16; e += 256) {
        int i, v;
        if (COLS) { i = e >> 4; v = e & 15; } else { v = e / np; i = e - v * np; }
        if (i < n && v0 + v < nvec) {
            const double x = (ident && i < v0 + v) ? 0.0 : Xs[i * PT + v];
            if (COLS) X[size_t(i) * ldx + v0 + v] = x;
            else X[size_t(v0 + v) * ldx + i] = x;
        }
    }
}

template <bool COLS, int TMAX>
__global__ void __launch_bounds__(256) k_trsm16(const double* __restrict__ L, const double* __restrict__ Dinv, int dld,
                                                int n, const double* __restrict__ Y, size_t ldy, double* __restrict__ X,
                                                size_t ldx, int nvec) {
    trsm16_body<COLS, TMAX>(L, Dinv, dld, n, Y, ldy, X, ldx, nvec, int(blockIdx.x) * 16, false);
}

template <int TMAX>
__global__ void __launch_bounds__(256) k_trinv_batched(const TrinvBatch b, int dld) {
    const int i = blockIdx.y, n = b.n[i];
    if (int(blockIdx.x) * 16 >= n) return;
    trsm16_body<true, TMAX>(b.L[i], b.Dinv[i], dld, n, nullptr, 0, b.X[i], size_t(n), n, int(blockIdx.x) * 16, true);
}

__device__ __forceinline__ double wsum(double v) {
#pragma unroll
    for (int o = 32; o > 0; o >>= 1) v += __shfl_xor(v, o, 64);
    return v;
}

__device__ double bsum(double v, double* red) {
    const int lane = threadIdx.x & 63, w = threadIdx.x >> 6, nw = blockDim.x >> 6;
    v = wsum(v);
    __syncthreads();
    if (lane == 0) red[w] = v;
    __syncthreads();
    double s = 0.0;
    for (int i = 0; i < nw; ++i) s += red[i];
    return s;
}

__global__ void __launch_bounds__(1024) k_qrcp(double* __restrict__ W, int m, int n, double* __restrict__ vn1,
                                                double* __restrict__ vn2, int* __restrict__ jpvt, double* __restrict__ tau,
                                                double* __restrict__ Q, double* __restrict__ Cout, int* __restrict__ rank_out,
                                                int pivot, int abs_r00, int rank_rule) {
    __shared__ double red[16];
    __shared__ double sh_beta, sh_tau, sh_scale;
    __shared__ int sh_p;
    __shared__ double sh_val[16];
    __shared__ int sh_idx[16];
    const int tid = threadIdx.x, lane = tid & 63, wave = tid >> 6;
    const int kmax = min(m, n);
    const double tol3z = sqrt(1.1102230246251565e-16);
    for (int j = wave; j < n; j += 16) {
        const double* col = W + size_t(j) * m;
        double s = 0.0;
        for (int i = lane; i < m; i += 64) s += col[i] * col[i];
        s = wsum(s);
        if (lane == 0) {
            vn1[j] = sqrt(s);
            vn2[j] = vn1[j];
            jpvt[j] = j;
        }
    }
    __syncthreads();
    for (int k = 0; k < kmax; ++k) {
        if (!pivot) {
            if (tid == 0) sh_p = k;
            __syncthreads();
        } else {
        double best = -1.0;
        int bi = n;
        for (int j = k + tid; j < n; j += 1024) {
            const double v = vn1[j];
            if (v > best || (v == best && j < bi)) { best = v; bi = j; }
        }
#pragma unroll
        for (int o = 32; o > 0; o >>= 1) {
            const double ov = __shfl_xor(best, o, 64);
            const int oi = __shfl_xor(bi, o, 64);
            if (ov > best || (ov == best && oi < bi)) { best = ov; bi = oi; }
        }
        if (lane == 0) { sh_val[wave] = best; sh_idx[wave] = bi; }
        __syncthreads();
        if (tid == 0) {
            double bv = -1.0;
            int b = n;
            for (int w = 0; w < 16; ++w)
                if (sh_val[w] > bv || (sh_val[w] == bv && sh_idx[w] < b)) { bv = sh_val[w]; b = sh_idx[w]; }
            sh_p = b;
        }
        __syncthreads();
        }
        const int p = (sh_p >= k && sh_p < n) ? sh_p : k;
        if (p != k) {
            double* ck = W + size_t(k) * m;
            double* cp = W + size_t(p) * m;
            for (int i = tid; i < m; i += 1024) {
                const double t = ck[i];
                ck[i] = cp[i];
                cp[i] = t;
            }
            __syncthreads();
            if (tid == 0) {
                const int t = jpvt[p]; jpvt[p] = jpvt[k]; jpvt[k] = t;
                vn1[p] = vn1[k];
                vn2[p] = vn2[k];
            }
        }
        __syncthreads();
        double* ck = W + size_t(k) * m;
        double s = 0.0;
        for (int i = k + 1 + tid; i < m; i += 1024) s += ck[i] * ck[i];
        const double xnorm = sqrt(bsum(s, red));
        if (tid == 0) {
            const double alpha = ck[k];
            if (m - k <= 1 || xnorm == 0.0) {
                sh_tau = 0.0;
                sh_beta = alpha;
            } else {
                const double beta = -copysign(hypot(alpha, xnorm), alpha);
                sh_tau = (beta - alpha) / beta;
                sh_beta = beta;
                sh_scale = 1.0 / (alpha - beta);
            }
        }
        __syncthreads();
        const double tk = sh_tau;
        if (tk != 0.0) {
            const double sc = sh_scale;
            for (int i = k + 1 + tid; i < m; i += 1024) ck[i] *= sc;
        }
        __syncthreads();
        if (tid == 0) {
            ck[k] = sh_beta;
            tau[k] = tk;
        }
        __syncthreads();
        if (tk != 0.0) {
            for (int j = k + 1 + wave; j < n; j += 16) {
                double* cj = W + size_t(j) * m;
                double d = (lane == 0) ? cj[k] : 0.0;
                for (int i = k + 1 + lane; i < m; i += 64) d += ck[i] * cj[i];
                d = wsum(d) * tk;
                if (lane == 0) cj[k] -= d;
                for (int i = k + 1 + lane; i < m; i += 64) cj[i] -= d * ck[i];
            }
        }
        __syncthreads();
        for (int j = k + 1 + wave; j < n; j += 16) {
            const double v1 = vn1[j];
            if (v1 != 0.0) {
                const double* cj = W + size_t(j) * m;
                double temp = fabs(cj[k]) / v1;
                temp = fmax(0.0, 1.0 - temp * temp);
                const double r12 = v1 / vn2[j];
                const double temp2 = temp * r12 * r12;
                if (temp2 <= tol3z) {
                    double s2 = 0.0;
                    for (int i = k + 1 + lane; i < m; i += 64) s2 += cj[i] * cj[i];
                    s2 = wsum(s2);
                    if (lane == 0) {
                        const double nv = (k + 1 < m) ? sqrt(s2) : 0.0;
                        vn1[j] = nv;
                        vn2[j] = nv;
                    }
                } else if (lane == 0) {
                    vn1[j] = v1 * sqrt(temp);
                }
            }
        }
        __syncthreads();
    }
    __shared__ int sh_rank;
    if (tid == 0) {
        const double r00 = abs_r00 ? fabs(W[0]) : W[0];
        int rank = kmax;
        if (rank_rule) {
            for (rank = 1; rank <= kmax; ++rank) {
                if (rank == kmax || fabs(W[size_t(rank) * m + rank]) < 16.0 * 2.220446049250313e-16 * r00) break;
            }
        }
        sh_rank = rank;
        rank_out[0] = rank;
    }
    __syncthreads();
    const int rank = sh_rank;
    for (int e = tid; e < rank * n; e += 1024) {
        const int row = e / n, col = e % n;
        Cout[size_t(row) * n + jpvt[col]] = (row <= col) ? W[size_t(col) * m + row] : 0.0;
    }
    for (int e = tid; e < m * kmax; e += 1024) {
        const int i = e / kmax, j = e % kmax;
        Q[e] = (i == j) ? 1.0 : 0.0;
    }
    __syncthreads();
    for (int i = kmax - 1; i >= 0; --i) {
        const double ti = tau[i];
        if (ti == 0.0) continue;
        const double* v = W + size_t(i) * m;
        for (int j = i + wave; j < kmax; j += 16) {
            double d = (lane == 0) ? Q[size_t(i) * kmax + j] : 0.0;
            for (int r = i + 1 + lane; r < m; r += 64) d += v[r] * Q[size_t(r) * kmax + j];
            d = wsum(d) * ti;
            if (lane == 0) Q[size_t(i) * kmax + j] -= d;
            for (int r = i + 1 + lane; r < m; r += 64) Q[size_t(r) * kmax + j] -= d * v[r];
        }
        __syncthreads();
    }
}

__global__ void __launch_bounds__(1024) k_jacobi(double* __restrict__ W, int p, int q, double* __restrict__ J,
                                                  int max_sweeps, double tol, int* __restrict__ sweeps_out) {
    __shared__ int rotated;
    __shared__ int perm[PMAX + 2];
    const int tid = threadIdx.x, lane = tid & 63, wave = tid >> 6;
    const int P = (p + 1) & ~1;
    for (int e = tid; e < p * p; e += 1024) J[e] = ((e / p) == (e % p)) ? 1.0 : 0.0;
    for (int i = tid; i < P; i += 1024) perm[i] = i;
    __syncthreads();
    int sweep = 0;
    for (; sweep < max_sweeps; ++sweep) {
        if (tid == 0) rotated = 0;
        __syncthreads();
        for (int round = 0; round < P - 1; ++round) {
            for (int t = wave; t < P / 2; t += 16) {
                int i = perm[t], j = perm[P - 1 - t];
                if (i >= p || j >= p) continue;
                if (i > j) { const int s = i; i = j; j = s; }
                double* wi = W + size_t(i) * q;
                double* wj = W + size_t(j) * q;
                double a = 0, b = 0, c = 0;
                for (int k = lane; k < q; k += 64) {
                    const double x = wi[k], y = wj[k];
                    a += x * x; b += y * y; c += x * y;
                }
                a = wsum(a); b = wsum(b); c = wsum(c);
                if (fabs(c) > tol * sqrt(a * b) && c != 0.0) {
                    const double zeta = (b - a) / (2.0 * c);
                    const double t_ = copysign(1.0, zeta) / (fabs(zeta) + sqrt(1.0 + zeta * zeta));
                    const double cs = 1.0 / sqrt(1.0 + t_ * t_);
                    const double sn = cs * t_;
                    const double tau = sn / (1.0 + cs);
                    for (int k = lane; k < q; k += 64) {
                        const double x = wi[k], y = wj[k];
                        wi[k] = x - sn * (y + tau * x);
                        wj[k] = y + sn * (x - tau * y);
                    }
                    double* ji = J + size_t(i) * p;
                    double* jj = J + size_t(j) * p;
                    for (int k = lane; k < p; k += 64) {
                        const double x = ji[k], y = jj[k];
                        ji[k] = x - sn * (y + tau * x);
                        jj[k] = y + sn * (x - tau * y);
                    }
                    if (lane == 0) rotated = 1;
                }
            }
            __syncthreads();
            if (tid == 0) {
                const int last = perm[P - 1];
                for (int s = P - 1; s > 1; --s) perm[s] = perm[s - 1];
                perm[1] = last;
            }
            __syncthreads();
        }
        if (!rotated) break;
    }
    if (tid == 0) sweeps_out[0] = (sweep < max_sweeps) ? sweep + 1 : -1;
}

__global__ void __launch_bounds__(1024) k_svd_finish(const double* __restrict__ Wr, int p, int q, const double* __restrict__ J,
                                                      double* __restrict__ U, double* __restrict__ S, double* __restrict__ Vt) {
    __shared__ double sn[PMAX];
    __shared__ int rk[PMAX];
    const int tid = threadIdx.x, lane = tid & 63, wave = tid >> 6;
    for (int i = wave; i < p; i += 16) {
        const double* w = Wr + size_t(i) * q;
        double s = 0.0;
        for (int k = lane; k < q; k += 64) s += w[k] * w[k];
        s = wsum(s);
        if (lane == 0) sn[i] = sqrt(s);
    }
    __syncthreads();
    for (int i = tid; i < p; i += 1024) {
        int r = 0;
        const double si = sn[i];
        for (int j = 0; j < p; ++j) r += (sn[j] > si) || (sn[j] == si && j < i);
        rk[i] = r;
    }
    __syncthreads();
    for (int i = tid; i < p; i += 1024) S[rk[i]] = sn[i];
    for (int e = tid; e < p * q; e += 1024) {
        const int i = e / q, k = e % q;
        const double s = sn[i];
        Vt[size_t(rk[i]) * q + k] = (s > 0.0) ? Wr[e] / s : 0.0;
    }
    for (int e = tid; e < p * p; e += 1024) {
        const int i = e / p, r = e % p;
        U[size_t(r) * p + rk[i]] = J[e];
    }
}

static int dinv_ld(int n) { return n <= PR_TMAX * 16 ? 16 : 32; }
size_t dinv_elems(int n) { return dinv_ld(n) == 16 ? size_t((n + 15) / 16) * 256 : size_t(n + 32) * 32; }

void potrf(xrs_handle_t h, double* G, int n, double shift_rel, double* Dinv, int* status_dev, double* info_dev) {
    XRS_REQUIRE(n >= 1 && n <= PMAX, "potrf: n out of range for the single-workgroup kernel");
    KernelTimer timer(h, XRS_KFAM_QR, double(n) * n * n / 3.0, 16.0 * double(n) * n);
    if (dinv_ld(n) == 16) {
        hipLaunchKernelGGL(k_potrf_rr, dim3(1), dim3(XRS_POTRF_RR_THREADS), 0, h->stream, G, n, shift_rel, Dinv, status_dev, info_dev);
        check_launch("k_potrf_rr");
    } else {
        hipLaunchKernelGGL(k_potrf, dim3(1), dim3(POT_THREADS), 0, h->stream, G, n, shift_rel, Dinv, status_dev, info_dev);
        check_launch("k_potrf");
    }
}

void potrf_batched(xrs_handle_t h, const PotrfBatch& b, int count) {
    XRS_REQUIRE(count >= 0 && count <= kPotrfBatchMax, "potrf_batched: batch too large");
    if (count == 0) return;
    PotrfBatch small{}, large{};
    int ns = 0, nl = 0;
    double fl_s = 0.0, fl_l = 0.0;
    for (int i = 0; i < count; ++i) {
        XRS_REQUIRE(b.n[i] >= 1 && b.n[i] <= PMAX, "potrf_batched: n out of range");
        const bool rr = dinv_ld(b.n[i]) == 16;
        PotrfBatch& d = rr ? small : large;
        int& c = rr ? ns : nl;
        XRS_REQUIRE(b.G[i] != nullptr || (rr && b.src[i] != nullptr), "potrf_batched: no input / output");
        d.src[c] = b.src[i];
        d.G[c] = b.G[i];
        d.Dinv[c] = b.Dinv[i];
        d.shift[c] = b.shift[i];
        d.n[c] = b.n[i];
        d.slot[c] = i;
        (rr ? fl_s : fl_l) += double(b.n[i]) * b.n[i] * b.n[i] / 3.0;
        ++c;
    }
    small.status = b.status;
    large.status = b.status;
    if (ns) {
        KernelTimer timer(h, XRS_KFAM_QR, fl_s, 0.0);
        hipLaunchKernelGGL(k_potrf_rr_batched, dim3(ns), dim3(XRS_POTRF_RR_THREADS), 0, h->stream, small);
        check_launch("k_potrf_rr_batched");
    }
    if (nl) {
        KernelTimer timer(h, XRS_KFAM_QR, fl_l, 0.0);
        hipLaunchKernelGGL(k_potrf32_batched, dim3(nl), dim3(POT_THREADS), 0, h->stream, large);
        check_launch("k_potrf32_batched");
    }
}

void trsm(xrs_handle_t h, bool cols, const double* L, const double* Dinv, int n, const double* Y, size_t ldy, double* X,
          size_t ldx, int nvec) {
    if (nvec <= 0) return;
    XRS_REQUIRE(n >= 1 && n <= PMAX, "trsm: n out of range");
    KernelTimer timer(h, XRS_KFAM_QR, double(n) * n * nvec, 8.0 * (2.0 * double(n) * nvec + double(n) * n));
    const unsigned blocks = unsigned((nvec + 15) / 16);
    const int dld = dinv_ld(n);
#define XRS_TRSM(C_, T_) \
    hipLaunchKernelGGL((k_trsm16<C_, T_>), dim3(blocks), dim3(256), 0, h->stream, L, Dinv, dld, n, Y, ldy, X, ldx, nvec)
    if (n <= 256) {
        if (cols) XRS_TRSM(true, 16); else XRS_TRSM(false, 16);
    } else {
        if (cols) XRS_TRSM(true, 32); else XRS_TRSM(false, 32);
    }
#undef XRS_TRSM
    check_launch("k_trsm16");
}

void trinv_batched(xrs_handle_t h, const TrinvBatch& b, int count) {
    XRS_REQUIRE(count >= 0 && count <= kTrinvBatchMax, "trinv_batched: batch too large");
    for (int big = 0; big < 2; ++big) {
        TrinvBatch g{};
        int c = 0, nmax = 0;
        double fl = 0.0;
        for (int i = 0; i < count; ++i) {
            XRS_REQUIRE(b.n[i] >= 1 && b.n[i] <= PMAX, "trinv_batched: n out of range");
            if ((dinv_ld(b.n[i]) == 32) != bool(big)) continue;
            g.L[c] = b.L[i];
            g.Dinv[c] = b.Dinv[i];
            g.X[c] = b.X[i];
            g.n[c] = b.n[i];
            nmax = std::max(nmax, b.n[i]);
            fl += double(b.n[i]) * b.n[i] * b.n[i];
            ++c;
        }
        if (c == 0) continue;
        KernelTimer timer(h, XRS_KFAM_QR, fl, 0.0);
        const dim3 grid(unsigned((nmax + 15) / 16), unsigned(c));
        if (big) hipLaunchKernelGGL((k_trinv_batched<32>), grid, dim3(256), 0, h->stream, g, 32);
        else hipLaunchKernelGGL((k_trinv_batched<16>), grid, dim3(256), 0, h->stream, g, 16);
        check_launch("k_trinv_batched");
    }
}

size_t qrcp(xrs_handle_t h, const double* A, size_t m, size_t n, double* Q, double* C, bool pivot, bool abs_r00,
            bool rank_rule) {
    XRS_REQUIRE(m >= 1 && n >= 1, "qrcp: empty matrix");
    XRS_REQUIRE(m < (1u << 24) && n < (1u << 24), "qrcp: matrix too large");
    const size_t kmax = std::min(m, n);
    DevBuf W(h, m * n * 8), vn(h, 2 * n * 8), jp(h, n * 4 + 64), tau(h, kmax * 8), rk(h, 64);
    transpose(h, W.d(), A, m, n);
    {
        KernelTimer timer(h, XRS_KFAM_QR, 4.0 * double(m) * n * kmax, 8.0 * 4.0 * double(m) * n);
        hipLaunchKernelGGL(k_qrcp, dim3(1), dim3(1024), 0, h->stream, W.d(), int(m), int(n), vn.d(), vn.d() + n, jp.as<int>(),
                           tau.d(), Q, C, rk.as<int>(), int(pivot), int(abs_r00), int(rank_rule));
        check_launch("k_qrcp");
    }
    int r = 0;
    read_status(h, rk.as<int>(), 1, &r);
    return size_t(r);
}

void jacobi_svd_rows(xrs_handle_t h, const double* W, int p, int q, double* U, double* S, double* Vt) {
    XRS_REQUIRE(p >= 1 && p <= PMAX && p <= q, "jacobi_svd_rows: need 1 <= p <= min(q, 512)");
    DevBuf st(h, 64);
    auto one_workgroup = [&](int) {
        DevBuf Wc(h, size_t(p) * q * 8), J(h, size_t(p) * p * 8);
        XRS_HIP(hipMemcpyAsync(Wc.d(), W, size_t(p) * q * 8, hipMemcpyDeviceToDevice, h->stream));
        KernelTimer timer(h, XRS_KFAM_SVD, 8.0 * double(p) * p * (p + q), 0.0);
        hipLaunchKernelGGL(k_jacobi, dim3(1), dim3(1024), 0, h->stream, Wc.d(), p, q, J.d(), 60, 4.0 * 2.220446049250313e-16,
                           st.as<int>());
        check_launch("k_jacobi");
        hipLaunchKernelGGL(k_svd_finish, dim3(1), dim3(1024), 0, h->stream, Wc.d(), p, q, J.d(), U, S, Vt);
        check_launch("k_svd_finish");
    };
    if (!jacobi_usv_fits(p, q)) return one_workgroup(1);
    jacobi_usv(h, W, q, false, p, q, U, p, S, Vt, q, st.as<int>(), 60);
    jacobi_settle(h, st.as<int>(), p, q, one_workgroup);
}

}
```

### xerus_amd/csrc/smallla.hpp

```cpp
#pragma once
#include <functional>
#include <vector>

#include "elementwise.hpp"

namespace xrs {

constexpr int kSmallMax = 512;

void potrf(xrs_handle_t h, double* G, int n, double shift_rel, double* Dinv, int* status_dev, double* info_dev = nullptr);
constexpr int kPotrfBatchMax = 48;
struct PotrfBatch {
    const double* src[kPotrfBatchMax];
    double* G[kPotrfBatchMax];
    double* Dinv[kPotrfBatchMax];
    double shift[kPotrfBatchMax];
    int n[kPotrfBatchMax];
    int slot[kPotrfBatchMax];
    int* status;
};
void potrf_batched(xrs_handle_t h, const PotrfBatch& b, int count);
size_t dinv_elems(int n);
constexpr int kTrinvBatchMax = 64;
struct TrinvBatch {
    const double* L[kTrinvBatchMax];
    const double* Dinv[kTrinvBatchMax];
    double* X[kTrinvBatchMax];
    int n[kTrinvBatchMax];
};
void trinv_batched(xrs_handle_t h, const TrinvBatch& b, int count);
void trsm(xrs_handle_t h, bool cols, const double* L, const double* Dinv, int n, const double* Y, size_t ldy, double* X,
          size_t ldx, int nvec);
size_t qrcp(xrs_handle_t h, const double* A, size_t m, size_t n, double* Q, double* C, bool pivot, bool abs_r00,
            bool rank_rule);
void jacobi_svd_rows(xrs_handle_t h, const double* W, int p, int q, double* U, double* S, double* Vt);

void jacobi_vt(xrs_handle_t h, const double* W, int ldw, bool trans, int p, int q, double* S, double* Vt, int ldvt,
               int* status_dev, int max_sweeps = 40, int kernel = 0, bool stamps = false, bool early = false);
bool jacobi_vt_fits_lds(int p, int q);
bool jacobi_usv_fits(int p, int q);
void jacobi_usv(xrs_handle_t h, const double* W, int ldw, bool trans, int p, int q, double* U, int ldu, double* S, double* Vt, int ldvt,
                int* status_dev, int max_sweeps = 40, bool early = false);
bool sym_eig_top_fits(int n, int kk);
void sym_eig_top(xrs_handle_t h, const double* A, int lda, int n, int kk, double* lam, double* S, double* Ut, int ldu, int* status_dev);
void sym_tridiag(xrs_handle_t h, const double* A, int lda, int n, double* d, double* e);
int svd_bidiag_mode();
bool svd_bidiag(xrs_handle_t h, const double* A, int n, double* U, double* S, double* Vt, double* diag = nullptr);
void jacobi_right_vectors(xrs_handle_t h, const double* F, int g, bool lower, double* S, double* Vt, int* status_dev,
                          int max_sweeps = 40, bool early = false);

int jacobi_settle(xrs_handle_t h, int* status_dev, int p, int q, const std::function<void(int kernel)>& rerun);

struct OrthResult {
    bool certified;
    double cert_ratio;
    bool robust;
};

OrthResult orthogonalize(xrs_handle_t h, const double* A, size_t m, size_t n, bool wide, double* Q, double* RL);

size_t qc(xrs_handle_t h, const double* A, size_t m, size_t n, double* Q, double* C);
size_t cq(xrs_handle_t h, const double* A, size_t m, size_t n, double* C, double* Q);
void qr(xrs_handle_t h, const double* A, size_t m, size_t n, double* Q, double* R);
void rq(xrs_handle_t h, const double* A, size_t m, size_t n, double* R, double* Q);
void svd(xrs_handle_t h, const double* A, size_t m, size_t n, double* U, double* S, double* Vt);

void solve_dense(xrs_handle_t h, double* X, const double* A, size_t m, size_t n, const double* B, size_t p);
void svd_solve(xrs_handle_t h, double* X, const double* A, size_t m, size_t n, const double* B, size_t p);
bool chol_blocked(xrs_handle_t h, const double* A, size_t n, double* L, std::vector<DevBuf>& Z);
void chol_solve(xrs_handle_t h, const double* L, const std::vector<DevBuf>& Z, size_t n, const double* B, size_t p, double* X);
int chol_full_blocks(size_t n);
void chol_full(xrs_handle_t h, const double* A, size_t n, double shift_rel, double* L, double* Z, int* status);

void transpose(xrs_handle_t h, double* out, const double* in, size_t rows, size_t cols);
int read_status(xrs_handle_t h, const int* status_dev, int count, int* host_out);

}
```

Baseline: 38590 GFLOP/s.

## Split blocked Cholesky into dedicated panel wave and trailing-update worker waves

Replaces the right-looking and lookahead tile Cholesky kernels with one variant where wave 0 factors the next diagonal block while the remaining waves apply the trailing MFMA updates, using double-buffered LDS panels and diagonal tiles. Trailing updates are grouped four tiles at a time to issue independent MFMA chains. It also adds a batched potrf C API that returns traces. The aim is to hide the serial diagonal-factor latency behind the update work, at the cost of one fewer worker wave and roughly double the LDS footprint.

```diff
diff --git a/include/xerus_amd.h b/include/xerus_amd.h
--- a/include/xerus_amd.h
+++ b/include/xerus_amd.h
@@ -75,6 +75,8 @@
 int xrs_svd_rows_vt(xrs_handle_t handle, double* S, double* Vt, int* sweeps, const double* A, size_t p, size_t q, int kernel);
 int xrs_sym_tridiag(xrs_handle_t handle, double* d, double* e, const double* A, size_t n);
 int xrs_sym_eig_top(xrs_handle_t handle, double* lam, double* Ut, int* status, const double* A, size_t n, size_t kk);
+int xrs_potrf_batched(xrs_handle_t handle, size_t count, const double* const* src, const size_t* n, const double* shift_rel,
+                      double* const* L, double* const* Dinv, int* status, double* trace);
 
 
 int xrs_tt_move_core(xrs_handle_t handle, size_t d, const size_t* n, size_t* r, double** cores,
diff --git a/xerus_amd/capi.py b/xerus_amd/capi.py
--- a/xerus_amd/capi.py
+++ b/xerus_amd/capi.py
@@ -52,6 +52,8 @@
     "xrs_solve_least_squares": (C.c_int, [_DP, _DP, _DP, _SZ, _SZ, _DP, _SZ]),
     "xrs_svd_rows_vt": (C.c_int, [_DP, _DP, _DP, C.POINTER(C.c_int), _DP, _SZ, _SZ, C.c_int]),
     "xrs_sym_eig_top": (C.c_int, [_DP, _DP, _DP, C.POINTER(C.c_int), _DP, _SZ, _SZ]),
+    "xrs_potrf_batched": (C.c_int, [_DP, _SZ, C.POINTER(_DP), C.POINTER(_SZ), C.POINTER(C.c_double), C.POINTER(_DP),
+                                    C.POINTER(_DP), C.POINTER(C.c_int), C.POINTER(C.c_double)]),
     "xrs_sym_tridiag": (C.c_int, [_DP, _DP, _DP, _DP, _SZ]),
     "xrs_tt_entrywise_product": (C.c_int, [_DP, _SZ, C.POINTER(_SZ), C.POINTER(_SZ), C.POINTER(_DP), C.POINTER(_SZ), C.POINTER(_DP),
                                            C.c_double, C.POINTER(_DP)]),
@@ -369,6 +371,19 @@
         _check("xrs_sym_eig_top", self.lib.xrs_sym_eig_top(self.h, _DP(lam.ptr), _DP(Ut.ptr), C.byref(st), _DP(A.ptr), n, kk))
         return lam, Ut, st.value
 
+    def potrf_batched(self, jobs):
+        cnt = len(jobs)
+        ns = [int(n) for _, n, _ in jobs]
+        L = [self.empty((n, n)) for n in ns]
+        Dinv = [self.empty(((n + 15) // 16, 16, 16) if n <= 256 else (n + 32, 32)) for n in ns]
+        st, tr = np.zeros(cnt, dtype=np.intc), np.zeros(cnt, dtype=np.float64)
+        _check("xrs_potrf_batched", self.lib.xrs_potrf_batched(
+            self.h, cnt, (_DP * cnt)(*[_DP(s.ptr) for s, _, _ in jobs]), (_SZ * cnt)(*ns),
+            (C.c_double * cnt)(*[float(t) for _, _, t in jobs]), (_DP * cnt)(*[_DP(x.ptr) for x in L]),
+            (_DP * cnt)(*[_DP(x.ptr) for x in Dinv]), st.ctypes.data_as(C.POINTER(C.c_int)),
+            tr.ctypes.data_as(C.POINTER(C.c_double))))
+        return L, Dinv, st, tr
+
     def sym_tridiag(self, A: "DeviceArray"):
         n = A.shape[0]
         d, e = self.empty((n,)), self.empty((n,))
diff --git a/xerus_amd/csrc/linalg.hip b/xerus_amd/csrc/linalg.hip
--- a/xerus_amd/csrc/linalg.hip
+++ b/xerus_amd/csrc/linalg.hip
@@ -511,6 +511,43 @@
     });
 }
 
+int xrs_potrf_batched(xrs_handle_t h, size_t count, const double* const* src, const size_t* n, const double* shift_rel,
+                      double* const* L, double* const* Dinv, int* status, double* trace) {
+    return guarded([&] {
+        XRS_REQUIRE(h && src && n && shift_rel && L && Dinv && status && trace, "null argument");
+        if (count == 0) return;
+        for (size_t i = 0; i < count; ++i)
+            XRS_REQUIRE(src[i] && L[i] && Dinv[i] && n[i] >= 1 && n[i] <= size_t(kSmallMax),
+                        "xrs_potrf_batched: need src, L, Dinv and 1 <= n <= 512 for every job");
+        fence_readers(h);
+        DevBuf st(h, count * sizeof(int)), tr(h, count * sizeof(double));
+        XRS_HIP(hipMemsetAsync(st.d(), 0, count * sizeof(int), h->stream));
+        XRS_HIP(hipMemsetAsync(tr.d(), 0, count * sizeof(double), h->stream));
+        if (count == 1) {
+            XRS_HIP(hipMemcpyAsync(L[0], src[0], n[0] * n[0] * sizeof(double), hipMemcpyDeviceToDevice, h->stream));
+            potrf(h, L[0], int(n[0]), shift_rel[0], Dinv[0], st.as<int>(), tr.as<double>());
+        } else {
+            for (size_t b0 = 0; b0 < count; b0 += size_t(kPotrfBatchMax)) {
+                PotrfBatch pb{};
+                const int c = int(std::min(size_t(kPotrfBatchMax), count - b0));
+                for (int i = 0; i < c; ++i) {
+                    const size_t e = b0 + size_t(i);
+                    pb.src[i] = src[e];
+                    pb.G[i] = L[e];
+                    pb.Dinv[i] = Dinv[e];
+                    pb.shift[i] = shift_rel[e];
+                    pb.n[i] = int(n[e]);
+                }
+                pb.status = st.as<int>() + b0;
+                pb.info = tr.as<double>() + b0;
+                potrf_batched(h, pb, c);
+            }
+        }
+        read_status(h, st.as<int>(), int(count), status);
+        XRS_HIP(hipMemcpy(trace, tr.d(), count * sizeof(double), hipMemcpyDeviceToHost));
+    });
+}
+
 int xrs_sym_tridiag(xrs_handle_t h, double* d, double* e, const double* A, size_t n) {
     return guarded([&] {
         XRS_REQUIRE(h && d && e && A, "null argument");
diff --git a/xerus_amd/csrc/smallla.hip b/xerus_amd/csrc/smallla.hip
--- a/xerus_amd/csrc/smallla.hip
+++ b/xerus_amd/csrc/smallla.hip
@@ -188,7 +188,6 @@
 constexpr int PR_THREADS = 512;
 constexpr int PR_WAVES = PR_THREADS / 64;
 constexpr int PR_TMAX = 16;
-constexpr int PR_SLOTS = (PR_TMAX * (PR_TMAX + 1) / 2 + PR_WAVES - 1) / PR_WAVES;
 constexpr int PT = 17;
 constexpr int PTILE = 16 * PT;
 
@@ -210,9 +209,6 @@
 
 #ifdef XRS_POTRF_STAMPS
 __device__ long long* g_potrf_stamps;
-#define PSTAMP(i) do { if (threadIdx.x == 0) g_potrf_stamps[i] = __builtin_amdgcn_s_memtime(); } while (0)
-#else
-#define PSTAMP(i) do { } while (0)
 #endif
 template <int K>
 __device__ __forceinline__ double row_bcast_d(double v) {
@@ -258,9 +254,6 @@
     int bad = 0;
     factor_all<0>(a, w, dsh, lane, valid, bad);
     wave_lds_sync();
-#ifdef XRS_POTRF_STAMPS
-    if (lane == 0) g_potrf_stamps[1000 + blockIdx.x] = __builtin_amdgcn_s_memtime();
-#endif
     if (lane < 16) {
 #pragma unroll
         for (int c = 0; c < 16; ++c) Dt[r * PT + c] = (c <= r) ? a[c] : 0.0;
@@ -282,56 +275,88 @@
     return bad;
 }
 
+constexpr int CP_WORKERS = PR_WAVES - 1;
+constexpr int CP_SLOTS = (PR_TMAX * (PR_TMAX + 1) / 2 + CP_WORKERS - 1) / CP_WORKERS;
+constexpr int CP_GROUP = 4;
+
+#ifdef XRS_POTRF_STAMPS
+#define CPSTAMP(t, k) do { if (lane == 0 && blockIdx.x == 0) g_potrf_stamps[((t) + 1) * 64 + wave * 8 + (k)] = __builtin_amdgcn_s_memtime(); } while (0)
+#else
+#define CPSTAMP(t, k) do { } while (0)
+#endif
+
+template <int S>
+__device__ __forceinline__ void cp_trail_one(d4 (&acc)[CP_SLOTS], const int (&ti)[CP_SLOTS], const int (&tk)[CP_SLOTS],
+                                             const double* Pbuf, int oa) {
+    const char* pa = reinterpret_cast<const char*>(Pbuf + ti[S] * PTILE) + oa;
+    const char* pb = reinterpret_cast<const char*>(Pbuf + tk[S] * PTILE) + oa;
+    double a[4], b[4];
+#pragma unroll
+    for (int c = 0; c < 4; ++c) {
+        a[c] = *reinterpret_cast<const double*>(pa + 32 * c);
+        b[c] = *reinterpret_cast<const double*>(pb + 32 * c);
+    }
+#pragma unroll
+    for (int c = 0; c < 4; ++c) acc[S] = __builtin_amdgcn_mfma_f64_16x16x4f64(-a[c], b[c], acc[S], 0, 0, 0);
+}
+
 template <int P>
-__device__ __forceinline__ void trail_pair(d4 (&acc)[PR_SLOTS], const int (&ti)[PR_SLOTS], const int (&tk)[PR_SLOTS], int j,
-                                           const double* Pbuf, int oa) {
-    const bool hi = tk[P] > j;
-    bool lo = false;
-    if constexpr (P > 0) lo = tk[P - 1] > j;
-    if (!hi && !lo) return;
-    auto op = [&](int tile, int c) -> double {
-        return *reinterpret_cast<const double*>(reinterpret_cast<const char*>(Pbuf + max(tile, 0) * PTILE) + oa + 32 * c);
-    };
-    double a1[4], b1[4];
-#pragma unroll
-    for (int c = 0; c < 4; ++c) {
-        a1[c] = hi ? -op(ti[P], c) : 0.0;
-        b1[c] = hi ? op(tk[P], c) : 0.0;
-    }
-    if constexpr (P > 0) {
-        double a0[4], b0[4];
-#pragma unroll
-        for (int c = 0; c < 4; ++c) {
-            a0[c] = lo ? -op(ti[P - 1], c) : 0.0;
-            b0[c] = lo ? op(tk[P - 1], c) : 0.0;
-        }
-#pragma unroll
-        for (int c = 0; c < 4; ++c) {
-            acc[P] = __builtin_amdgcn_mfma_f64_16x16x4f64(a1[c], b1[c], acc[P], 0, 0, 0);
-            acc[P - 1] = __builtin_amdgcn_mfma_f64_16x16x4f64(a0[c], b0[c], acc[P - 1], 0, 0, 0);
-        }
+__device__ __forceinline__ void cp_trail_group(d4 (&acc)[CP_SLOTS], const int (&ti)[CP_SLOTS], const int (&tk)[CP_SLOTS],
+                                               int kmin, int kmax, const double* Pbuf, int oa) {
+    constexpr int N = (P + 1 < CP_GROUP) ? P + 1 : CP_GROUP;
+    bool on[N];
+    bool any = false, all = true;
+#pragma unroll
+    for (int u = 0; u < N; ++u) {
+        on[u] = tk[P - u] >= kmin && tk[P - u] <= kmax;
+        any = any || on[u];
+        all = all && on[u];
+    }
+    if (!any) return;
+    if (all) {
+        double a[N][4], b[N][4];
+#pragma unroll
+        for (int u = 0; u < N; ++u) {
+            const char* pa = reinterpret_cast<const char*>(Pbuf + ti[P - u] * PTILE) + oa;
+            const char* pb = reinterpret_cast<const char*>(Pbuf + tk[P - u] * PTILE) + oa;
+#pragma unroll
+            for (int c = 0; c < 4; ++c) {
+                a[u][c] = *reinterpret_cast<const double*>(pa + 32 * c);
+                b[u][c] = *reinterpret_cast<const double*>(pb + 32 * c);
+            }
+        }
+#pragma unroll
+        for (int c = 0; c < 4; ++c)
+#pragma unroll
+            for (int u = 0; u < N; ++u)
+                acc[P - u] = __builtin_amdgcn_mfma_f64_16x16x4f64(-a[u][c], b[u][c], acc[P - u], 0, 0, 0);
     } else {
-#pragma unroll
-        for (int c = 0; c < 4; ++c) acc[P] = __builtin_amdgcn_mfma_f64_16x16x4f64(a1[c], b1[c], acc[P], 0, 0, 0);
+        if (on[0]) cp_trail_one<P>(acc, ti, tk, Pbuf, oa);
+        if constexpr (N > 1) { if (on[1]) cp_trail_one<P - 1>(acc, ti, tk, Pbuf, oa); }
+        if constexpr (N > 2) { if (on[2]) cp_trail_one<P - 2>(acc, ti, tk, Pbuf, oa); }
+        if constexpr (N > 3) { if (on[3]) cp_trail_one<P - 3>(acc, ti, tk, Pbuf, oa); }
     }
 }
 
 template <int P>
-__device__ __forceinline__ void trail_all(d4 (&acc)[PR_SLOTS], const int (&ti)[PR_SLOTS], const int (&tk)[PR_SLOTS], int j,
-                                          const double* Pbuf, int oa) {
+__device__ __forceinline__ void cp_trail_all(d4 (&acc)[CP_SLOTS], const int (&ti)[CP_SLOTS], const int (&tk)[CP_SLOTS],
+                                             int kmin, int kmax, const double* Pbuf, int oa) {
     if constexpr (P >= 0) {
-        trail_pair<P>(acc, ti, tk, j, Pbuf, oa);
-        trail_all<P - 2>(acc, ti, tk, j, Pbuf, oa);
-    }
-}
-
-__device__ __forceinline__ void potrf_rr_body(double* __restrict__ G, int n, double shift_rel, double* __restrict__ Dinv,
+        cp_trail_group<P>(acc, ti, tk, kmin, kmax, Pbuf, oa);
+        cp_trail_all<P - CP_GROUP>(acc, ti, tk, kmin, kmax, Pbuf, oa);
+    }
+}
+static_assert(CP_GROUP <= 4);
+
+__device__ __forceinline__ void potrf_cp_body(double* __restrict__ G, int n, double shift_rel, double* __restrict__ Dinv,
                                               int* __restrict__ status, double* __restrict__ info,
                                               const double* __restrict__ src = nullptr) {
     const double* __restrict__ S = src != nullptr ? src : G;
-    __shared__ double Dt[PTILE];
-    __shared__ double Di[PTILE];
-    __shared__ double P[PR_TMAX * PTILE];
+    __shared__ double Dt[2 * PTILE];
+    __shared__ double Di[2 * PTILE];
+    __shared__ double Hs[2 * 2 * PTILE];
+    __shared__ double Ws[2 * PTILE];
+    __shared__ double P[2 * PR_TMAX * PTILE];
     __shared__ double ivs[16];
     __shared__ double red[PR_WAVES];
     __shared__ int fail;
@@ -341,7 +366,6 @@
     const int T = (n + 15) >> 4;
     const int ntiles = T * (T + 1) / 2;
     if (tid == 0) fail = 0;
-    PSTAMP(0);
     double tr = 0.0;
     for (int i = tid; i < n; i += PR_THREADS) tr += S[size_t(i) * n + i];
 #pragma unroll
@@ -353,209 +377,6 @@
     for (int w = 0; w < PR_WAVES; ++w) tr += red[w];
     if (tid == 0 && info) info[0] = tr;
     const double shift = shift_rel * tr;
-
-    int ti[PR_SLOTS], tk[PR_SLOTS];
-    d4 acc[PR_SLOTS];
-#pragma unroll
-    for (int s = 0; s < PR_SLOTS; ++s) {
-        const int t = s * PR_WAVES + wave;
-        int i = -1, k = -1;
-        if (t < ntiles) {
-            int start = 0;
-            k = 0;
-            while (t >= start + (T - k)) { start += T - k; ++k; }
-            i = k + (t - start);
-        }
-        ti[s] = i;
-        tk[s] = k;
-#pragma unroll
-        for (int q = 0; q < 4; ++q) {
-            const int row = min(max(16 * i + lg + 4 * q, 0), n - 1), col = min(max(16 * k + lr, 0), n - 1);
-            acc[s][q] = S[size_t(row) * n + col];
-        }
-    }
-#pragma unroll
-    for (int s = 0; s < PR_SLOTS; ++s)
-#pragma unroll
-        for (int q = 0; q < 4; ++q) {
-            const int row = 16 * ti[s] + lg + 4 * q, col = 16 * tk[s] + lr;
-            const bool inside = ti[s] >= 0 && row < n && col < n;
-            const double pad = (row == col) ? 1.0 : 0.0;
-            acc[s][q] = inside ? acc[s][q] + ((row == col) ? shift : 0.0) : pad;
-        }
-
-    for (int j = 0; j < T; ++j) {
-        int oc = (lg * PT + lr) * 8, oa = (lr * PT + lg) * 8;
-        asm volatile("" : "+v"(oc), "+v"(oa));
-        auto cpos = [&](double* base, int q) -> double* {
-            return reinterpret_cast<double*>(reinterpret_cast<char*>(base) + oc) + 4 * q * PT;
-        };
-        auto apos = [&](const double* base, int c) -> const double* {
-            return reinterpret_cast<const double*>(reinterpret_cast<const char*>(base) + oa) + 4 * c;
-        };
-#pragma unroll
-        for (int s = 0; s < PR_SLOTS; ++s)
-            if (ti[s] == j && tk[s] == j) {
-#pragma unroll
-                for (int q = 0; q < 4; ++q) *cpos(Dt, q) = acc[s][q];
-            }
-        __syncthreads();
-        PSTAMP(2 + 4 * j);
-        if (wave == 0) {
-            const int bad = diag_factor16(Dt, Di, ivs, Dinv + size_t(j) * 256, lane, n - 16 * j);
-            if (lane == 0 && bad && fail == 0) fail = 16 * j + bad;
-        }
-        __syncthreads();
-        PSTAMP(3 + 4 * j);
-#pragma unroll
-        for (int s = 0; s < PR_SLOTS; ++s) {
-            if (tk[s] != j) continue;
-            if (ti[s] == j) {
-#pragma unroll
-                for (int q = 0; q < 4; ++q) acc[s][q] = *cpos(Dt, q);
-                continue;
-            }
-            double* Pi = P + ti[s] * PTILE;
-#pragma unroll
-            for (int q = 0; q < 4; ++q) *cpos(Pi, q) = acc[s][q];
-            wave_lds_sync();
-            d4 rr = {0.0, 0.0, 0.0, 0.0};
-#pragma unroll
-            for (int c = 0; c < 4; ++c) rr = __builtin_amdgcn_mfma_f64_16x16x4f64(*apos(Pi, c), *apos(Di, c), rr, 0, 0, 0);
-            wave_lds_sync();
-#pragma unroll
-            for (int q = 0; q < 4; ++q) *cpos(Pi, q) = rr[q];
-            acc[s] = rr;
-        }
-        __syncthreads();
-        PSTAMP(4 + 4 * j);
-        trail_all<PR_SLOTS - 1>(acc, ti, tk, j, P, oa);
-    }
-    __syncthreads();
-    PSTAMP(1);
-    int sg = lg, sr = lr;
-    asm volatile("" : "+v"(sg), "+v"(sr));
-#pragma unroll
-    for (int s = 0; s < PR_SLOTS; ++s) {
-        if (ti[s] < 0 || G == nullptr) continue;
-#pragma unroll
-        for (int q = 0; q < 4; ++q) {
-            const int row = 16 * ti[s] + sg + 4 * q, col = 16 * tk[s] + sr;
-            if (row < n && col < n) {
-                G[size_t(row) * n + col] = (col <= row) ? acc[s][q] : 0.0;
-                if (ti[s] != tk[s]) G[size_t(col) * n + row] = 0.0;
-            }
-        }
-    }
-    __syncthreads();
-    if (tid == 0) status[0] = fail;
-}
-
-constexpr int LA_THREADS = PR_THREADS;
-constexpr int LA_WAVES = LA_THREADS / 64;
-constexpr int LA_SLOTS = PR_SLOTS;
-
-template <int P>
-__device__ __forceinline__ void la_trail_pair(d4 (&acc)[LA_SLOTS], const int (&ti)[LA_SLOTS], const int (&tk)[LA_SLOTS],
-                                              int kmin, int kmax, const double* Pbuf, int oa) {
-    const bool hi = tk[P] >= kmin && tk[P] <= kmax;
-    bool lo = false;
-    if constexpr (P > 0) lo = tk[P - 1] >= kmin && tk[P - 1] <= kmax;
-    if (!hi && !lo) return;
-    auto op = [&](int tile, int c) -> double {
-        return *reinterpret_cast<const double*>(reinterpret_cast<const char*>(Pbuf + max(tile, 0) * PTILE) + oa + 32 * c);
-    };
-    double a1[4], b1[4];
-#pragma unroll
-    for (int c = 0; c < 4; ++c) {
-        a1[c] = hi ? -op(ti[P], c) : 0.0;
-        b1[c] = hi ? op(tk[P], c) : 0.0;
-    }
-    if constexpr (P > 0) {
-        double a0[4], b0[4];
-#pragma unroll
-        for (int c = 0; c < 4; ++c) {
-            a0[c] = lo ? -op(ti[P - 1], c) : 0.0;
-            b0[c] = lo ? op(tk[P - 1], c) : 0.0;
-        }
-#pragma unroll
-        for (int c = 0; c < 4; ++c) {
-            acc[P] = __builtin_amdgcn_mfma_f64_16x16x4f64(a1[c], b1[c], acc[P], 0, 0, 0);
-            acc[P - 1] = __builtin_amdgcn_mfma_f64_16x16x4f64(a0[c], b0[c], acc[P - 1], 0, 0, 0);
-        }
-    } else {
-#pragma unroll
-        for (int c = 0; c < 4; ++c) acc[P] = __builtin_amdgcn_mfma_f64_16x16x4f64(a1[c], b1[c], acc[P], 0, 0, 0);
-    }
-}
-
-template <int P>
-__device__ __forceinline__ void la_trail_all(d4 (&acc)[LA_SLOTS], const int (&ti)[LA_SLOTS], const int (&tk)[LA_SLOTS],
-                                             int kmin, int kmax, const double* Pbuf, int oa) {
-    if constexpr (P >= 0) {
-        la_trail_pair<P>(acc, ti, tk, kmin, kmax, Pbuf, oa);
-        la_trail_all<P - 2>(acc, ti, tk, kmin, kmax, Pbuf, oa);
-    }
-}
-
-__device__ __forceinline__ void potrf_la_body(double* __restrict__ G, int n, double shift_rel, double* __restrict__ Dinv,
-                                              int* __restrict__ status, double* __restrict__ info,
-                                              const double* __restrict__ src = nullptr) {
-    const double* __restrict__ S = src != nullptr ? src : G;
-    __shared__ double Dt[PTILE];
-    __shared__ double Di[PTILE];
-    __shared__ double P[PR_TMAX * PTILE];
-    __shared__ double ivs[16];
-    __shared__ double red[LA_WAVES];
-    __shared__ int fail;
-    const int tid = threadIdx.x, lane = tid & 63;
-    const int wave = __builtin_amdgcn_readfirstlane(tid >> 6);
-    const int lr = lane & 15, lg = lane >> 4;
-    const int T = (n + 15) >> 4;
-    const int ntiles = T * (T + 1) / 2;
-    if (tid == 0) fail = 0;
-    PSTAMP(0);
-    double tr = 0.0;
-    for (int i = tid; i < n; i += LA_THREADS) tr += S[size_t(i) * n + i];
-#pragma unroll
-    for (int o = 32; o > 0; o >>= 1) tr += __shfl_xor(tr, o, 64);
-    if (lane == 0) red[wave] = tr;
-    __syncthreads();
-    tr = 0.0;
-#pragma unroll
-    for (int w = 0; w < LA_WAVES; ++w) tr += red[w];
-    if (tid == 0 && info) info[0] = tr;
-    const double shift = shift_rel * tr;
-
-    int ti[LA_SLOTS], tk[LA_SLOTS];
-    d4 acc[LA_SLOTS];
-#pragma unroll
-    for (int s = 0; s < LA_SLOTS; ++s) {
-        const int t = wave == 0 ? s : LA_SLOTS + s * (LA_WAVES - 1) + (wave - 1);
-        int i = -1, k = -1;
-        if (t < ntiles) {
-            int start = 0;
-            k = 0;
-            while (t >= start + (T - k)) { start += T - k; ++k; }
-            i = k + (t - start);
-        }
-        ti[s] = i;
-        tk[s] = k;
-#pragma unroll
-        for (int q = 0; q < 4; ++q) {
-            const int row = min(max(16 * i + lg + 4 * q, 0), n - 1), col = min(max(16 * k + lr, 0), n - 1);
-            acc[s][q] = S[size_t(row) * n + col];
-        }
-    }
-#pragma unroll
-    for (int s = 0; s < LA_SLOTS; ++s)
-#pragma unroll
-        for (int q = 0; q < 4; ++q) {
-            const int row = 16 * ti[s] + lg + 4 * q, col = 16 * tk[s] + lr;
-            const bool inside = ti[s] >= 0 && row < n && col < n;
-            const double pad = (row == col) ? 1.0 : 0.0;
-            acc[s][q] = inside ? acc[s][q] + ((row == col) ? shift : 0.0) : pad;
-        }
 
     int oc = (lg * PT + lr) * 8, oa = (lr * PT + lg) * 8;
     auto cpos = [&](double* base, int q) -> double* {
@@ -564,70 +385,175 @@
     auto apos = [&](const double* base, int c) -> const double* {
         return reinterpret_cast<const double*>(reinterpret_cast<const char*>(base) + oa) + 4 * c;
     };
-    auto publish_diag = [&](int j) {
-#pragma unroll
-        for (int s = 0; s < LA_SLOTS; ++s)
-            if (ti[s] == j && tk[s] == j) {
-#pragma unroll
-                for (int q = 0; q < 4; ++q) *cpos(Dt, q) = acc[s][q];
-            }
-    };
-    auto factor_diag = [&](int j) {
-        if (wave == 0) {
-            const int bad = diag_factor16(Dt, Di, ivs, Dinv + size_t(j) * 256, lane, n - 16 * j);
-            if (lane == 0 && bad && fail == 0) fail = 16 * j + bad;
-        }
-    };
-    publish_diag(0);
-    __syncthreads();
-    factor_diag(0);
-    __syncthreads();
-    for (int j = 0; j < T; ++j) {
-        asm volatile("" : "+v"(oc), "+v"(oa));
-        PSTAMP(2 + 4 * j);
-#pragma unroll
-        for (int s = 0; s < LA_SLOTS; ++s) {
-            if (tk[s] != j) continue;
-            if (ti[s] == j) {
-#pragma unroll
-                for (int q = 0; q < 4; ++q) acc[s][q] = *cpos(Dt, q);
-                continue;
-            }
-            double* Pi = P + ti[s] * PTILE;
-#pragma unroll
-            for (int q = 0; q < 4; ++q) *cpos(Pi, q) = acc[s][q];
-            wave_lds_sync();
-            d4 rr = {0.0, 0.0, 0.0, 0.0};
-#pragma unroll
-            for (int c = 0; c < 4; ++c) rr = __builtin_amdgcn_mfma_f64_16x16x4f64(*apos(Pi, c), *apos(Di, c), rr, 0, 0, 0);
-            wave_lds_sync();
-#pragma unroll
-            for (int q = 0; q < 4; ++q) *cpos(Pi, q) = rr[q];
-            acc[s] = rr;
-        }
-        __syncthreads();
-        if (j + 1 >= T) break;
-        PSTAMP(3 + 4 * j);
-        la_trail_all<LA_SLOTS - 1>(acc, ti, tk, j + 1, j + 1, P, oa);
-        publish_diag(j + 1);
-        __syncthreads();
-        PSTAMP(4 + 4 * j);
-        if (wave == 0) factor_diag(j + 1);
-        la_trail_all<LA_SLOTS - 1>(acc, ti, tk, j + 2, T - 1, P, oa);
-        __syncthreads();
-    }
-    PSTAMP(1);
-    int sg = lg, sr = lr;
-    asm volatile("" : "+v"(sg), "+v"(sr));
-#pragma unroll
-    for (int s = 0; s < LA_SLOTS; ++s) {
-        if (ti[s] < 0 || G == nullptr) continue;
-#pragma unroll
-        for (int q = 0; q < 4; ++q) {
-            const int row = 16 * ti[s] + sg + 4 * q, col = 16 * tk[s] + sr;
-            if (row < n && col < n) {
-                G[size_t(row) * n + col] = (col <= row) ? acc[s][q] : 0.0;
-                if (ti[s] != tk[s]) G[size_t(col) * n + row] = 0.0;
+    if (wave == 0) {
+        __builtin_amdgcn_s_setprio(3);
+        for (int t = -1; t < T; ++t) {
+            const int cur = t & 1, nxt = cur ^ 1;
+            const double* Pprev = P + nxt * (PR_TMAX * PTILE);
+            CPSTAMP(t, 0);
+            if (t + 1 < T) {
+                double* Dn = Dt + nxt * PTILE;
+                if (t < 0) {
+#pragma unroll
+                    for (int q = 0; q < 4; ++q) {
+                        const int row = lg + 4 * q, col = lr;
+                        const double v = S[unsigned(min(row, n - 1) * n + min(col, n - 1))];
+                        const double pad = (row == col) ? 1.0 : 0.0;
+                        *cpos(Dn, q) = (row < n && col < n) ? v + ((row == col) ? shift : 0.0) : pad;
+                    }
+                    wave_lds_sync();
+                } else {
+                    double* Hc = Hs + cur * (2 * PTILE);
+                    d4 sub, dg;
+#pragma unroll
+                    for (int q = 0; q < 4; ++q) {
+                        sub[q] = *cpos(Hc, q);
+                        dg[q] = *cpos(Hc + PTILE, q);
+                    }
+                    if (t >= 1) {
+                        double a[4], b[4];
+#pragma unroll
+                        for (int c = 0; c < 4; ++c) {
+                            a[c] = *apos(Pprev + (t + 1) * PTILE, c);
+                            b[c] = *apos(Pprev + t * PTILE, c);
+                        }
+#pragma unroll
+                        for (int c = 0; c < 4; ++c) {
+                            sub = __builtin_amdgcn_mfma_f64_16x16x4f64(-a[c], b[c], sub, 0, 0, 0);
+                            dg = __builtin_amdgcn_mfma_f64_16x16x4f64(-a[c], a[c], dg, 0, 0, 0);
+                        }
+                    }
+#pragma unroll
+                    for (int q = 0; q < 4; ++q) *cpos(Ws, q) = sub[q];
+                    wave_lds_sync();
+                    d4 rr = {0.0, 0.0, 0.0, 0.0};
+#pragma unroll
+                    for (int c = 0; c < 4; ++c)
+                        rr = __builtin_amdgcn_mfma_f64_16x16x4f64(*apos(Ws, c), *apos(Di + cur * PTILE, c), rr, 0, 0, 0);
+#pragma unroll
+                    for (int q = 0; q < 4; ++q) *cpos(Ws + PTILE, q) = rr[q];
+                    wave_lds_sync();
+#pragma unroll
+                    for (int c = 0; c < 4; ++c) {
+                        const double l = *apos(Ws + PTILE, c);
+                        dg = __builtin_amdgcn_mfma_f64_16x16x4f64(-l, l, dg, 0, 0, 0);
+                    }
+#pragma unroll
+                    for (int q = 0; q < 4; ++q) *cpos(Dn, q) = dg[q];
+                    wave_lds_sync();
+                }
+                CPSTAMP(t, 1);
+                const int bad = diag_factor16(Dn, Di + nxt * PTILE, ivs, Dinv + size_t(t + 1) * 256, lane, n - 16 * (t + 1));
+                if (lane == 0 && bad && fail == 0) fail = 16 * (t + 1) + bad;
+            }
+            CPSTAMP(t, 2);
+            __syncthreads();
+            CPSTAMP(t, 4);
+        }
+        __builtin_amdgcn_s_setprio(0);
+    } else {
+        int ti[CP_SLOTS], tk[CP_SLOTS];
+        d4 acc[CP_SLOTS];
+#pragma unroll
+        for (int s = 0; s < CP_SLOTS; ++s) {
+            const int t = s * CP_WORKERS + (wave - 1);
+            int i = -1, k = -1;
+            if (t < ntiles) {
+                int start = 0;
+                k = 0;
+                while (t >= start + (T - k)) { start += T - k; ++k; }
+                i = k + (t - start);
+            }
+            ti[s] = i;
+            tk[s] = k;
+        }
+#pragma unroll
+        for (int h = 0; h < CP_SLOTS; h += CP_SLOTS / 2) {
+#pragma unroll
+            for (int s = h; s < h + CP_SLOTS / 2; ++s)
+#pragma unroll
+                for (int q = 0; q < 4; ++q) {
+                    const int row = min(max(16 * ti[s] + lg + 4 * q, 0), n - 1), col = min(max(16 * tk[s] + lr, 0), n - 1);
+                    acc[s][q] = S[unsigned(row * n + col)];
+                }
+            int fg = lg, fr = lr;
+            asm volatile("" : "+v"(fg), "+v"(fr));
+#pragma unroll
+            for (int s = h; s < h + CP_SLOTS / 2; ++s)
+#pragma unroll
+                for (int q = 0; q < 4; ++q) {
+                    const int row = 16 * ti[s] + fg + 4 * q, col = 16 * tk[s] + fr;
+                    const bool inside = ti[s] >= 0 && row < n && col < n;
+                    const double pad = (row == col) ? 1.0 : 0.0;
+                    acc[s][q] = inside ? acc[s][q] + ((row == col) ? shift : 0.0) : pad;
+                }
+            __builtin_amdgcn_sched_barrier(0);
+        }
+        for (int t = -1; t < T; ++t) {
+            asm volatile("" : "+v"(oc), "+v"(oa));
+            const int cur = t & 1, nxt = cur ^ 1;
+            double* Pcur = P + cur * (PR_TMAX * PTILE);
+            const double* Pprev = P + nxt * (PR_TMAX * PTILE);
+            CPSTAMP(t, 0);
+            if (t >= 1) cp_trail_all<CP_SLOTS - 1>(acc, ti, tk, t, t, Pprev, oa);
+            CPSTAMP(t, 1);
+            if (t >= 0) {
+#pragma unroll
+                for (int s = 0; s < CP_SLOTS; ++s) {
+                    if (tk[s] != t) continue;
+                    if (ti[s] == t) {
+#pragma unroll
+                        for (int q = 0; q < 4; ++q) acc[s][q] = *cpos(Dt + cur * PTILE, q);
+                    } else {
+#pragma unroll
+                        for (int q = 0; q < 4; ++q) *cpos(Pcur + ti[s] * PTILE, q) = acc[s][q];
+                    }
+                }
+                wave_lds_sync();
+                double dj[4];
+#pragma unroll
+                for (int c = 0; c < 4; ++c) dj[c] = *apos(Di + cur * PTILE, c);
+#pragma unroll
+                for (int s = 0; s < CP_SLOTS; ++s) {
+                    if (tk[s] != t || ti[s] == t) continue;
+                    double* Pi = Pcur + ti[s] * PTILE;
+                    double a[4];
+#pragma unroll
+                    for (int c = 0; c < 4; ++c) a[c] = *apos(Pi, c);
+                    d4 rr = {0.0, 0.0, 0.0, 0.0};
+#pragma unroll
+                    for (int c = 0; c < 4; ++c) rr = __builtin_amdgcn_mfma_f64_16x16x4f64(a[c], dj[c], rr, 0, 0, 0);
+                    wave_lds_sync();
+#pragma unroll
+                    for (int q = 0; q < 4; ++q) *cpos(Pi, q) = rr[q];
+                    acc[s] = rr;
+                }
+            }
+            CPSTAMP(t, 2);
+            if (t >= 1) cp_trail_all<CP_SLOTS - 1>(acc, ti, tk, t + 1, T - 1, Pprev, oa);
+#pragma unroll
+            for (int s = 0; s < CP_SLOTS; ++s)
+                if (ti[s] == t + 2 && tk[s] >= t + 1) {
+                    double* Hn = Hs + nxt * (2 * PTILE) + (tk[s] - (t + 1)) * PTILE;
+#pragma unroll
+                    for (int q = 0; q < 4; ++q) *cpos(Hn, q) = acc[s][q];
+                }
+            CPSTAMP(t, 3);
+            __syncthreads();
+            CPSTAMP(t, 4);
+        }
+        int sg = lg, sr = lr;
+        asm volatile("" : "+v"(sg), "+v"(sr));
+#pragma unroll
+        for (int s = 0; s < CP_SLOTS; ++s) {
+            if (ti[s] < 0 || G == nullptr) continue;
+#pragma unroll
+            for (int q = 0; q < 4; ++q) {
+                const int row = 16 * ti[s] + sg + 4 * q, col = 16 * tk[s] + sr;
+                if (row < n && col < n) {
+                    G[size_t(row) * n + col] = (col <= row) ? acc[s][q] : 0.0;
+                    if (ti[s] != tk[s]) G[size_t(col) * n + row] = 0.0;
+                }
             }
         }
     }
@@ -635,26 +561,20 @@
     if (tid == 0) status[0] = fail;
 }
 
-#ifdef XRS_POTRF_NO_LOOKAHEAD
-#define XRS_POTRF_RR_BODY potrf_rr_body
-#else
-#define XRS_POTRF_RR_BODY potrf_la_body
-#endif
-#define XRS_POTRF_RR_THREADS PR_THREADS
-__global__ void __launch_bounds__(XRS_POTRF_RR_THREADS) k_potrf_rr(double* __restrict__ G, int n, double shift_rel,
+__global__ void __launch_bounds__(PR_THREADS) k_potrf_rr(double* __restrict__ G, int n, double shift_rel,
                                                          double* __restrict__ Dinv, int* __restrict__ status,
                                                          double* __restrict__ info) {
-    XRS_POTRF_RR_BODY(G, n, shift_rel, Dinv, status, info);
+    potrf_cp_body(G, n, shift_rel, Dinv, status, info);
 }
 
 __global__ void __launch_bounds__(POT_THREADS) k_potrf32_batched(PotrfBatch b) {
     const int i = blockIdx.x;
-    potrf32_body(b.G[i], b.n[i], b.shift[i], b.Dinv[i], b.status + b.slot[i], nullptr, b.src[i]);
-}
-
-__global__ void __launch_bounds__(XRS_POTRF_RR_THREADS) k_potrf_rr_batched(PotrfBatch b) {
+    potrf32_body(b.G[i], b.n[i], b.shift[i], b.Dinv[i], b.status + b.slot[i], b.info ? b.info + b.slot[i] : nullptr, b.src[i]);
+}
+
+__global__ void __launch_bounds__(PR_THREADS) k_potrf_rr_batched(PotrfBatch b) {
     const int i = blockIdx.x;
-    XRS_POTRF_RR_BODY(b.G[i], b.n[i], b.shift[i], b.Dinv[i], b.status + b.slot[i], nullptr, b.src[i]);
+    potrf_cp_body(b.G[i], b.n[i], b.shift[i], b.Dinv[i], b.status + b.slot[i], b.info ? b.info + b.slot[i] : nullptr, b.src[i]);
 }
 
 template <bool COLS, int TMAX>
@@ -1061,7 +981,7 @@
     XRS_REQUIRE(n >= 1 && n <= PMAX, "potrf: n out of range for the single-workgroup kernel");
     KernelTimer timer(h, XRS_KFAM_QR, double(n) * n * n / 3.0, 16.0 * double(n) * n);
     if (dinv_ld(n) == 16) {
-        hipLaunchKernelGGL(k_potrf_rr, dim3(1), dim3(XRS_POTRF_RR_THREADS), 0, h->stream, G, n, shift_rel, Dinv, status_dev, info_dev);
+        hipLaunchKernelGGL(k_potrf_rr, dim3(1), dim3(PR_THREADS), 0, h->stream, G, n, shift_rel, Dinv, status_dev, info_dev);
         check_launch("k_potrf_rr");
     } else {
         hipLaunchKernelGGL(k_potrf, dim3(1), dim3(POT_THREADS), 0, h->stream, G, n, shift_rel, Dinv, status_dev, info_dev);
@@ -1092,9 +1012,11 @@
     }
     small.status = b.status;
     large.status = b.status;
+    small.info = b.info;
+    large.info = b.info;
     if (ns) {
         KernelTimer timer(h, XRS_KFAM_QR, fl_s, 0.0);
-        hipLaunchKernelGGL(k_potrf_rr_batched, dim3(ns), dim3(XRS_POTRF_RR_THREADS), 0, h->stream, small);
+        hipLaunchKernelGGL(k_potrf_rr_batched, dim3(ns), dim3(PR_THREADS), 0, h->stream, small);
         check_launch("k_potrf_rr_batched");
     }
     if (nl) {
diff --git a/xerus_amd/csrc/smallla.hpp b/xerus_amd/csrc/smallla.hpp
--- a/xerus_amd/csrc/smallla.hpp
+++ b/xerus_amd/csrc/smallla.hpp
@@ -18,6 +18,7 @@
     int n[kPotrfBatchMax];
     int slot[kPotrfBatchMax];
     int* status;
+    double* info;
 };
 void potrf_batched(xrs_handle_t h, const PotrfBatch& b, int count);
 size_t dinv_elems(int n);
```

Result: no change. 38990 GFLOP/s, median of 3 (+1.0%).
